# alvinwan/neural-backed-decision-trees

Measured on AMD Instinct MI355X. Metric: images/sec training SoftNBDT WRN28x10 CIFAR10, higher is better.
Workload: dtype bf16; 1 GPU; WideResNet-28-10 + SoftTreeSupLoss (induced-wrn28_10_cifar10, 10 leaves), CIFAR10-shaped 3x32x32, SGD m=0.9 wd=5e-4; batch_per_gpu=512, global_batch=512, parallelism=dp1

## Files before the change

### include/nbdt_hip.h

```cpp
#ifndef NBDT_HIP_H
#define NBDT_HIP_H

#include <stdint.h>

#ifdef __cplusplus
extern "C" {
#endif

#define NBDT_OK 0
#define NBDT_EINVAL (-1)
#define NBDT_EHIP (-2)
#define NBDT_ENOMEM (-3)

#define NBDT_F32 0
#define NBDT_BF16 1
#define NBDT_F16 2

const char* nbdt_last_error(void);
const char* nbdt_debug_last_igemm(void);
const char* nbdt_debug_last_igemm_full(void);
const char* nbdt_debug_last_wgrad(void);
int nbdt_version(void);
int nbdt_set_deterministic(int32_t on);
int nbdt_get_deterministic(void);
int nbdt_set_wgrad_store_epilogue(int32_t on);
int nbdt_get_wgrad_store_epilogue(void);
int nbdt_set_reserved_cus(int32_t n);
int nbdt_get_reserved_cus(void);
int nbdt_set_stream_nt_min_bytes(int64_t bytes);
int64_t nbdt_get_stream_nt_min_bytes(void);
int nbdt_debug_last_stream_nt(void);
int nbdt_device_count(void);

int nbdt_weight_tile_batched(const void* src_bf16, const int64_t* table, int32_t n, int64_t total_tiles,
                             void* dst_bf16, void* stream);

typedef struct nbdt_tree nbdt_tree;
int nbdt_tree_create(int device, int num_classes, int num_inodes, int root,
                     const int32_t* node_off, const int32_t* slot_off, const int32_t* slot_cls,
                     const int32_t* cls_off, const int32_t* cls_slot, const int32_t* slot_next,
                     nbdt_tree** out);
int nbdt_tree_destroy(nbdt_tree* t);
int nbdt_tree_max_depth(const nbdt_tree* t);


int nbdt_soft_forward(const nbdt_tree* t, const void* z, int ztype, int64_t B, int64_t ldz,
                      float* P, void* stream);
int nbdt_soft_backward(const nbdt_tree* t, const void* z, int ztype, int64_t B, int64_t ldz,
                       const float* gP, float* gz, void* stream);
int nbdt_soft_tree_loss(const nbdt_tree* t, const void* z, int ztype, int64_t B, int64_t ldz,
                        const int64_t* y, float w_xent, float w_tree, float grad_scale,
                        float* row_loss, float* loss, float* gz, void* stream);
int nbdt_head_soft_tree_loss(const nbdt_tree* t, const float* pooled, const float* W, const float* bias, int64_t B,
                             int32_t K, const int64_t* y, float w_xent, float w_tree, float grad_scale,
                             float* row_loss, float* loss, float* z_out, float* gpooled, float* gW, float* gb,
                             void* stream);

int nbdt_hard_tree_loss(const nbdt_tree* t, const void* z, int ztype, int64_t B, int64_t ldz,
                        const int64_t* y, float w_xent, float w_node, float grad_scale,
                        float* row_loss, float* loss, float* gz, void* stream);
int nbdt_soft_tree_loss_ex(const nbdt_tree* t, const void* z, int ztype, int64_t B, int64_t ldz, const int64_t* y,
                           const float* tprob, int64_t ldt, float smoothing, float w_xent, float w_tree,
                           float grad_scale, float* row_loss, float* loss, float* gz, void* stream);
int nbdt_hard_tree_loss_ex(const nbdt_tree* t, const void* z, int ztype, int64_t B, int64_t ldz, const int64_t* y,
                           float smoothing, float w_xent, float w_node, float grad_scale, float* row_loss, float* loss,
                           float* gz, void* stream);
int nbdt_node_logits_backward(const nbdt_tree* t, const float* gs, int64_t B, float* gz, void* stream);
int nbdt_hard_forward(const nbdt_tree* t, const void* z, int ztype, int64_t B, int64_t ldz,
                      int64_t* pred, float* onehot, int32_t* path_node, int32_t* path_child,
                      float* path_prob, float* path_entropy, void* stream);
int nbdt_node_outputs(const nbdt_tree* t, const void* z, int ztype, int64_t B, int64_t ldz,
                      float* logits, float* probs, int64_t* preds, float* entropy, void* stream);

typedef struct nbdt_tree_stats {
  int64_t* totals;
  int64_t* confusion_net;
  int64_t* confusion_hard;
  int64_t* confusion_soft;
  int64_t* node_counts;
  int64_t* node_entropy;
  int64_t* first_error_depth;
} nbdt_tree_stats;
int nbdt_tree_stats_accumulate(const nbdt_tree* t, const void* z, int ztype, int64_t B, int64_t ldz,
                               const int64_t* y, const nbdt_tree_stats* stats, float* scores, void* stream);

typedef struct nbdt_conv_desc {
  int32_t B, gh, gw;
  int32_t cin, cout;
  int32_t ntaps;
  int32_t tap_off[9];
  int32_t w_tap[9];
  int32_t w_ntaps;
  int32_t in_bs, in_hs, in_ws, in_base;
  int32_t out_bs, out_hs, out_ws, out_base;
  int32_t accumulate;
  int32_t wide_tile;
  int32_t ksplit;
  uint64_t w_tiled;
} nbdt_conv_desc;
int nbdt_conv_plan(const nbdt_conv_desc* d, int32_t* form, int32_t* ksplit);
int nbdt_conv_igemm(const nbdt_conv_desc* d, const void* in, const void* w, void* out,
                    const void* residual, void* stream);

int nbdt_conv_igemm_multi(const nbdt_conv_desc* descs, int32_t n, const void* in, const void* w, void* out,
                          void* stream);

typedef struct nbdt_conv_seg_slice {
  int32_t tensor;
  int32_t ch0;
  int32_t ntaps;
  int32_t tap[9];
  int32_t w_matrix;
  int32_t w_off[9];
} nbdt_conv_seg_slice;
typedef struct nbdt_conv_seg_class {
  int32_t nslices;
  const nbdt_conv_seg_slice* slices;
  int32_t out_bs, out_hs, out_ws, out_base;
} nbdt_conv_seg_class;
#define NBDT_SEG_MAX_SLICES 64
typedef struct nbdt_conv_seg_desc {
  int32_t B, gh, gw;
  int32_t cout;
  int32_t ntensors;
  int32_t pix_stride[4];
  int32_t nmatrices;
  int32_t w_row_stride[4];
  int32_t nclasses;
  nbdt_conv_seg_class cls[4];
  int32_t tile;
  int32_t nbuf;
} nbdt_conv_seg_desc;
int nbdt_conv_seg_create(const nbdt_conv_seg_desc* d, void** plan);
int nbdt_conv_seg_destroy(void* plan);
int nbdt_conv_seg_info(void* plan, int32_t* tile, int32_t* nbuf, int32_t* steps, int32_t* max_rounds,
                       int64_t* w_tile_elems);
int nbdt_conv_seg_tile_weights(void* plan, const void* const* w, void* w_tiles, void* stream);
int nbdt_conv_seg(void* plan, const void* const* in, const void* w_tiles, void* out, const void* residual,
                  float* bn_partials, void* stream);
int nbdt_conv_seg_steps(void* plan, int32_t cls, int32_t* out8, int32_t max_steps, int32_t* npro);

int nbdt_conv_igemm_stats(const nbdt_conv_desc* d, const void* in, const void* w, void* out,
                          const void* residual, float* bn_partials, void* stream);

int nbdt_conv_igemm_bnbwd(const nbdt_conv_desc* d, const void* in, const void* w, void* out,
                          const void* bn_x, const float* save_mean, const float* save_rstd,
                          const float* gamma, const float* beta, float* bn_partials, void* stream);
int nbdt_conv_igemm_affine(const nbdt_conv_desc* d, const void* in, const void* w, void* out,
                           const void* residual, const float* scale, const float* shift, int32_t act,
                           void* stream);

int nbdt_conv_pw(const nbdt_conv_desc* d, const void* in, const void* w, void* out,
                 float* bn_partials , void* stream);

typedef struct nbdt_wgrad_desc {
  int32_t B, gh, gw;
  int32_t cin, cout;
  int32_t ntaps;
  int32_t tap_off[9];
  int32_t w_tap[9];
  int32_t w_ntaps;
  int32_t x_bs, x_hs, x_ws, x_base;
  int32_t g_bs, g_hs, g_ws, g_base;
  int32_t variant;
  int32_t cu_budget;
} nbdt_wgrad_desc;
int nbdt_conv_wgrad(const nbdt_wgrad_desc* d, const void* x, const void* gy, float* dw,
                    void* stream);
int nbdt_conv_wgrad_blocks(const nbdt_wgrad_desc* d);

int nbdt_weight_prep(const float* w, int32_t cout, int32_t taps, int32_t cin, void* w_bf16,
                     void* wd_bf16, void* stream);

int nbdt_weight_prep_batched(const float* flat, const int64_t* table, int32_t n_layers, int64_t total_tiles,
                             void* wd_flat, void* stream);

#define NBDT_BN_SLOTS 32
int nbdt_bn_stats(const void* x, int32_t B, int32_t H, int32_t W, int32_t C, float eps,
                  float momentum, float* running_mean, float* running_var, float* scratch,
                  float* save_mean, float* save_rstd, void* stream);
int nbdt_bn_finalize(int32_t B, int32_t H, int32_t W, int32_t C, float eps, float momentum,
                     float* running_mean, float* running_var, const float* bn_partials, float* save_mean,
                     float* save_rstd, void* stream);
int nbdt_bn_apply(const void* x, const float* save_mean, const float* save_rstd, const float* gamma,
                  const float* beta, const void* residual, int32_t relu, int32_t B, int32_t H,
                  int32_t W, int32_t C, void* y, void* stream);
int nbdt_bn_apply_s2d(const void* x, const float* save_mean, const float* save_rstd, const float* gamma,
                      const float* beta, int32_t relu, int32_t B, int32_t H, int32_t W, int32_t C, void* y,
                      void* stream);
int nbdt_bn_bwd_reduce(const void* gy, const void* y, const void* x, const float* save_mean,
                       const float* save_rstd, const float* gamma, const float* beta, int32_t relu,
                       int32_t B, int32_t H, int32_t W, int32_t C, float* scratch, float* dsum,
                       float* dgamma, float* dbeta, void* stream);
int nbdt_bn_bwd_fold(int32_t B, int32_t H, int32_t W, int32_t C, const float* bn_partials, float* dsum,
                     float* dgamma, float* dbeta, void* stream);
int nbdt_bn_bwd_apply(const void* gy, const void* y, const void* x, const float* save_mean,
                      const float* save_rstd, const float* gamma, const float* beta, const float* dsum,
                      const void* gx_add, int32_t relu, int32_t B, int32_t H, int32_t W, int32_t C,
                      void* gx, void* g_resid, void* stream);
int nbdt_bn_bwd_apply_cus(const void* gy, const void* x, const float* save_mean, const float* save_rstd,
                          const float* gamma, const float* beta, const float* dsum, const void* gx_add,
                          int32_t B, int32_t H, int32_t W, int32_t C, void* gx, int32_t cus, void* stream);
int nbdt_bn_bwd_reduce_cus(const void* gy, const void* x, const float* save_mean, const float* save_rstd,
                           const float* gamma, const float* beta, int32_t B, int32_t H, int32_t W, int32_t C,
                           float* scratch, float* dsum, float* dgamma, float* dbeta, int32_t cus, void* stream);
int nbdt_bn_bwd_cus(const void* gy, const void* x, const float* save_mean, const float* save_rstd, const float* gamma,
                    const float* beta, const void* gx_add, int32_t B, int32_t H, int32_t W, int32_t C, float* slots,
                    float* slots_other, float* dsum, float* dgamma, float* dbeta, void* gx, int32_t cus,
                    void* stream);
int nbdt_bn_relu_pool(const void* x, const float* save_mean, const float* save_rstd,
                      const float* gamma, const float* beta, int32_t B, int32_t H, int32_t W,
                      int32_t C, float* pooled, void* stream);
int nbdt_pool_bn_bwd_reduce(const float* gpooled, const void* x, const float* save_mean,
                            const float* save_rstd, const float* gamma, const float* beta,
                            int32_t B, int32_t H, int32_t W, int32_t C, float* scratch, float* dsum,
                            float* dgamma, float* dbeta, void* stream);
int nbdt_pool_bn_bwd_apply(const float* gpooled, const void* x, const float* save_mean,
                           const float* save_rstd, const float* gamma, const float* beta,
                           const float* dsum, int32_t B, int32_t H, int32_t W, int32_t C, void* gx,
                           void* stream);

#define NBDT_ACT_NONE 0
#define NBDT_ACT_RELU 1
#define NBDT_ACT_SWISH 2
int nbdt_bn_act_apply(const void* x, const float* save_mean, const float* save_rstd, const float* gamma,
                      const float* beta, int32_t act, const float* gate, const void* residual, int32_t B,
                      int32_t H, int32_t W, int32_t C, void* y, void* stream);
int nbdt_bn_act_pool(const void* x, const float* save_mean, const float* save_rstd, const float* gamma,
                     const float* beta, int32_t act, const void* mul, float scale, int32_t B, int32_t H,
                     int32_t W, int32_t C, float* out, void* stream);
int nbdt_bn_act_bwd(const void* gu, const float* gate, const float* gpool, const void* x,
                    const float* save_mean, const float* save_rstd, const float* gamma, const float* beta,
                    int32_t act, const void* gx_add, int32_t B, int32_t H, int32_t W, int32_t C,
                    float* scratch, float* dsum, float* dgamma, float* dbeta, void* gx, void* stream);
int nbdt_dwconv_fwd(const void* x, const float* w, int32_t B, int32_t H, int32_t W, int32_t C, int32_t k,
                    int32_t stride, void* y, float* bn_scratch , void* stream);
int nbdt_dwconv_bwd_data(const void* gy, const float* w, int32_t B, int32_t H, int32_t W, int32_t C,
                         int32_t k, int32_t stride, void* gx, void* stream);
int nbdt_dwconv_bwd_data_bn(const void* gy, const float* w, int32_t B, int32_t H, int32_t W, int32_t C, int32_t k,
                            void* gx, const void* bn_x, const float* save_mean, const float* save_rstd,
                            const float* gamma, const float* beta, float* scratch, void* stream);
int nbdt_bn_act_bwd_apply(const void* gu, const void* x, const float* save_mean, const float* save_rstd,
                          const float* gamma, const float* beta, int32_t act, const void* gx_add, int32_t B, int32_t H,
                          int32_t W, int32_t C, float* scratch, float* dsum, float* dgamma, float* dbeta, void* gx,
                          void* stream);
int nbdt_bn_act_se_sums(const void* gu, const void* x, const float* save_mean, const float* save_rstd,
                        const float* gamma, const float* beta, int32_t act, int32_t B, int32_t H, int32_t W, int32_t C,
                        float* sums, void* stream);
int nbdt_bn_act_se_bwd_apply(const void* gu, const float* gate, const float* gpool, float* sums, const void* x,
                             const float* save_mean, const float* save_rstd, const float* gamma, const float* beta,
                             int32_t act, int32_t B, int32_t H, int32_t W, int32_t C, float* dsum, float* dgamma,
                             float* dbeta, void* gx, void* stream);
int nbdt_dwconv_bwd_weight(const void* x, const void* gy, int32_t B, int32_t H, int32_t W, int32_t C,
                           int32_t k, int32_t stride, float* dw, void* stream);
int nbdt_se_gate_fwd(const float* pooled, const float* w1, const float* b1, const float* w2,
                     const float* b2, int32_t B, int32_t C, int32_t C_real, int32_t S, float* pre1,
                     float* gate, void* stream);
int nbdt_se_gate_bwd(const float* dgate, const float* gate, const float* pre1, const float* pooled,
                     const float* w1, const float* w2, int32_t B, int32_t C, int32_t C_real, int32_t S,
                     float* dpre2, float* dpre1, float* gpool, float* dw1, float* db1, float* dw2,
                     float* db2, void* stream);
int nbdt_se_param_grad(const float* dpre2, const float* dpre1, const float* pre1, const float* pooled,
                       int32_t B, int32_t C, int32_t C_real, int32_t S, float* dw1, float* db1, float* dw2,
                       float* db2, void* stream);
int nbdt_dropout_fwd(const float* x, int64_t n, float p, uint32_t seed, uint8_t* mask, float* y,
                     void* stream);
int nbdt_dropout_bwd(const float* gy, int64_t n, float p, const uint8_t* mask, float* gx, void* stream);

int nbdt_bn_act_apply_rows(const void* x, const float* save_mean, const float* save_rstd, const float* gamma,
                           const float* beta, int32_t act, const float* gate, const void* residual,
                           const float* row_scale, int32_t B, int32_t H, int32_t W, int32_t C, void* y, void* stream);
int nbdt_bn_act_bwd_rows(const void* gu, const float* row_scale, const float* gate, const float* gpool, const void* x,
                         const float* save_mean, const float* save_rstd, const float* gamma, const float* beta,
                         int32_t act, const void* gx_add, int32_t B, int32_t H, int32_t W, int32_t C, float* scratch,
                         float* dsum, float* dgamma, float* dbeta, void* gx, void* stream);
#define NBDT_SD_MAX_UNITS 64
int nbdt_stochastic_depth_draw(uint64_t seed, uint64_t stream_id, uint64_t counter, const float* prob,
                               const float* scale, int32_t U, int32_t B, float* table, void* stream);

int nbdt_ref_conv(const nbdt_conv_desc* d, const float* in, const float* w, float* out, const float* residual,
                  void* stream);
int nbdt_ref_wgrad(const nbdt_wgrad_desc* d, const float* x, const float* gy, float* dw, void* stream);
int nbdt_ref_conv_seg(void* plan, const float* const* in, const float* const* w, float* out, const float* residual,
                      void* stream);
int nbdt_ref_bn_stats(const float* x, int32_t B, int32_t H, int32_t W, int32_t C, float eps, float momentum,
                      float* running_mean, float* running_var, float* save_mean, float* save_rstd, float* partials,
                      void* stream);
int nbdt_ref_bn_apply(const float* x, const float* save_mean, const float* save_rstd, const float* gamma,
                      const float* beta, const float* residual, int32_t relu, int32_t B, int32_t H, int32_t W,
                      int32_t C, float* y, void* stream);
int nbdt_ref_bn_apply_s2d(const float* x, const float* save_mean, const float* save_rstd, const float* gamma,
                          const float* beta, int32_t relu, int32_t B, int32_t H, int32_t W, int32_t C, float* y,
                          void* stream);
int nbdt_ref_bn_bwd(const float* gy, const float* gpooled, const float* y, const float* x, const float* save_mean,
                    const float* save_rstd, const float* gamma, const float* beta, int32_t relu, const float* gx_add,
                    int32_t B, int32_t H, int32_t W, int32_t C, int32_t reduce, float* dsum, float* dgamma,
                    float* dbeta, float* gx, float* g_resid, void* stream);
int nbdt_ref_bn_relu_pool(const float* x, const float* save_mean, const float* save_rstd, const float* gamma,
                          const float* beta, int32_t B, int32_t H, int32_t W, int32_t C, float* pooled, void* stream);
int nbdt_ref_stem_conv(const float* img, const float* w, int32_t B, int32_t H, int32_t W, int32_t cout_real,
                       int32_t cpad, int32_t stride, float* out, void* stream);
int nbdt_ref_stem_wgrad(const float* img, const float* gy, int32_t B, int32_t H, int32_t W, int32_t cout_real,
                        int32_t cpad, int32_t stride, float* dw, void* stream);
int nbdt_ref_bn_act_apply(const float* x, const float* save_mean, const float* save_rstd, const float* gamma,
                          const float* beta, int32_t act, const float* gate, const float* residual, int32_t B, int32_t H,
                          int32_t W, int32_t C, float* y, void* stream);
int nbdt_ref_bn_act_pool(const float* x, const float* save_mean, const float* save_rstd, const float* gamma,
                         const float* beta, int32_t act, const float* mul, float scale, int32_t B, int32_t H, int32_t W,
                         int32_t C, float* out, void* stream);
int nbdt_ref_bn_act_bwd(const float* gu, const float* gate, const float* gpool, const float* x, const float* save_mean,
                        const float* save_rstd, const float* gamma, const float* beta, int32_t act, const float* gx_add,
                        int32_t B, int32_t H, int32_t W, int32_t C, float* dsum, float* dgamma, float* dbeta, float* gx,
                        void* stream);
int nbdt_ref_bn_act_apply_rows(const float* x, const float* save_mean, const float* save_rstd, const float* gamma,
                               const float* beta, int32_t act, const float* gate, const float* residual,
                               const float* row_scale, int32_t B, int32_t H, int32_t W, int32_t C, float* y,
                               void* stream);
int nbdt_ref_bn_act_bwd_rows(const float* gu, const float* row_scale, const float* gate, const float* gpool,
                             const float* x, const float* save_mean, const float* save_rstd, const float* gamma,
                             const float* beta, int32_t act, const float* gx_add, int32_t B, int32_t H, int32_t W,
                             int32_t C, float* dsum, float* dgamma, float* dbeta, float* gx, void* stream);
int nbdt_ref_dwconv_fwd(const float* x, const float* w, int32_t B, int32_t H, int32_t W, int32_t C, int32_t k,
// ... 159 lines not shown
```

### neural-backed-decision-trees_amd/csrc/bn.hip

```cpp
#include "common.h"

using namespace nbdt;

constexpr int kSlots = NBDT_BN_SLOTS;
constexpr int kMaxThreads = 256;

struct Layout {
  int c8, py, threads;
};
static Layout layout_for(int C) {
  Layout l;
  l.c8 = C / 8;
  l.py = kMaxThreads / l.c8;
  if (l.py < 1) l.py = 1;
  l.threads = l.c8 * l.py;
  return l;
}
static int grid_for(const PadGeom& g, const Layout& l, int pixels_per_thread) {
  long long want = ((long long)g.npix + (long long)l.py * pixels_per_thread - 1) / ((long long)l.py * pixels_per_thread);
  if (want < 1) want = 1;
  if (want > 2048) want = 2048;
  return (int)want;
}

template <int NQ>
__device__ __forceinline__ void block_fold_to_slots(float (&acc)[NQ][8], int cx, int py, int c8, int PY, int C,
                                                    float* scratch, float* lds, unsigned slot_mask) {
  float* mine = lds + ((size_t)py * c8 + cx) * (NQ * 8);
#pragma unroll
  for (int q = 0; q < NQ; ++q)
#pragma unroll
    for (int i = 0; i < 8; ++i) mine[q * 8 + i] = acc[q][i];
  __syncthreads();
  const int nch = c8 * 8, nthr = c8 * PY;
  for (int o = py * c8 + cx; o < NQ * nch; o += nthr) {
    const int q = o / nch, c = o - q * nch;
    const float* src = lds + (size_t)(c >> 3) * (NQ * 8) + q * 8 + (c & 7);
    float s = 0.f;
    for (int r = 0; r < PY; ++r) s += src[(size_t)r * c8 * (NQ * 8)];
    atomicAdd(scratch + ((size_t)(blockIdx.x & slot_mask) * NQ + q) * C + c, s);
  }
}

__global__ __launch_bounds__(kMaxThreads) void bn_stats_kernel(const bf16_t* __restrict__ x, PadGeom g, int c8,
                                                               int PY, float* __restrict__ scratch,
                                                               unsigned slot_mask) {
  extern __shared__ float lds[];
  const int cx = threadIdx.x % c8, py = threadIdx.x / c8;
  float acc[2][8];
#pragma unroll
  for (int i = 0; i < 8; ++i) acc[0][i] = acc[1][i] = 0.f;
  for (int p = blockIdx.x * PY + py; p < g.npix; p += gridDim.x * PY) {
    const u32x4_t v = *(const u32x4_t*)(x + pad_offset(g, p) + cx * 8);
    float f[8];
    unpack8(v, f);
#pragma unroll
    for (int i = 0; i < 8; ++i) {
      acc[0][i] += f[i];
      acc[1][i] += f[i] * f[i];
    }
  }
  block_fold_to_slots<2>(acc, cx, py, c8, PY, g.C, scratch, lds, slot_mask);
}

__global__ __launch_bounds__(256) void bn_finalize_kernel(float* __restrict__ scratch, int C, float n,
                                                          float eps, float momentum,
                                                          float* __restrict__ running_mean,
                                                          float* __restrict__ running_var,
                                                          float* __restrict__ save_mean,
                                                          float* __restrict__ save_rstd) {
  for (int c = blockIdx.x * 256 + threadIdx.x; c < C; c += gridDim.x * 256) {
    float s = 0.f, sq = 0.f;
#pragma unroll 8
    for (int k = 0; k < kSlots; ++k) {
      s += scratch[((size_t)k * 2 + 0) * C + c];
      sq += scratch[((size_t)k * 2 + 1) * C + c];
    }
#pragma unroll 8
    for (int k = 0; k < kSlots; ++k) {
      scratch[((size_t)k * 2 + 0) * C + c] = 0.f;
      scratch[((size_t)k * 2 + 1) * C + c] = 0.f;
    }
    const float mean = s / n;
    float var = sq / n - mean * mean;
    var = var > 0.f ? var : 0.f;
    save_mean[c] = mean;
    save_rstd[c] = rsqrtf(var + eps);
    if (running_mean) {
      running_mean[c] = (1.f - momentum) * running_mean[c] + momentum * mean;
      const float unbiased = n > 1.f ? var * n / (n - 1.f) : var;
      running_var[c] = (1.f - momentum) * running_var[c] + momentum * unbiased;
    }
  }
}

__global__ __launch_bounds__(256) void bn_bwd_finalize_kernel(float* __restrict__ scratch, int C,
                                                              float* __restrict__ dsum,
                                                              float* __restrict__ dgamma,
                                                              float* __restrict__ dbeta) {
  for (int c = blockIdx.x * 256 + threadIdx.x; c < C; c += gridDim.x * 256) {
    float s0 = 0.f, s1 = 0.f;
#pragma unroll 8
    for (int k = 0; k < kSlots; ++k) {
      s0 += scratch[((size_t)k * 2 + 0) * C + c];
      s1 += scratch[((size_t)k * 2 + 1) * C + c];
    }
#pragma unroll 8
    for (int k = 0; k < kSlots; ++k) {
      scratch[((size_t)k * 2 + 0) * C + c] = 0.f;
      scratch[((size_t)k * 2 + 1) * C + c] = 0.f;
    }
    dsum[c] = s0;
    dsum[C + c] = s1;
    if (dbeta) dbeta[c] += s0;
    if (dgamma) dgamma[c] += s1;
  }
}

template <bool RELU, bool HAS_RES, bool NT>
__global__ __launch_bounds__(kMaxThreads) void bn_apply_kernel(const bf16_t* __restrict__ x,
                                                               const float* __restrict__ mean,
                                                               const float* __restrict__ rstd,
                                                               const float* __restrict__ gamma,
                                                               const float* __restrict__ beta,
                                                               const bf16_t* __restrict__ res, PadGeom g, int c8,
                                                               int PY, bf16_t* __restrict__ y) {
  const int cx = threadIdx.x % c8, py = threadIdx.x / c8;
  float sc[8], sh[8];
#pragma unroll
  for (int i = 0; i < 8; ++i) {
    const int c = cx * 8 + i;
    sc[i] = gamma[c] * rstd[c];
    sh[i] = beta[c] - mean[c] * sc[i];
  }
  for (int p = blockIdx.x * PY + py; p < g.npix; p += gridDim.x * PY) {
    const int o = pad_offset(g, p) + cx * 8;
    float f[8];
    unpack8(ld16_stream<NT>(x + o), f);
    float r[8];
    if (HAS_RES) unpack8(ld16_stream<NT>(res + o), r);
#pragma unroll
    for (int i = 0; i < 8; ++i) {
      float v = f[i] * sc[i] + sh[i];
      if (HAS_RES) v += r[i];
      if (RELU) v = v > 0.f ? v : 0.f;
      f[i] = v;
    }
    *(u32x4_t*)(y + o) = pack8(f);
  }
}

template <bool RELU, bool POOL>
__global__ __launch_bounds__(kMaxThreads) void bn_bwd_reduce_kernel(const bf16_t* __restrict__ gy,
                                                                    const float* __restrict__ gpooled,
                                                                    const bf16_t* __restrict__ y,
                                                                    const bf16_t* __restrict__ x,
                                                                    const float* __restrict__ mean,
                                                                    const float* __restrict__ rstd,
                                                                    const float* __restrict__ gamma,
                                                                    const float* __restrict__ beta, PadGeom g,
                                                                    int c8, int PY, float* __restrict__ scratch,
                                                                    unsigned slot_mask) {
  extern __shared__ float lds[];
  const int cx = threadIdx.x % c8, py = threadIdx.x / c8;
  const bool maskx = POOL || (RELU && y == nullptr);
  float mu[8], rs[8], sc[8], sh[8];
#pragma unroll
  for (int i = 0; i < 8; ++i) {
    const int c = cx * 8 + i;
    mu[i] = mean[c];
    rs[i] = rstd[c];
    if (maskx) { sc[i] = gamma[c] * rs[i]; sh[i] = beta[c] - mu[i] * sc[i]; }
  }
  const float inv_hw = 1.f / (float)(g.H * g.W);
  const int hw = g.H * g.W;
  float acc[2][8];
#pragma unroll
  for (int i = 0; i < 8; ++i) acc[0][i] = acc[1][i] = 0.f;
  auto one = [&](int p, const u32x4_t vx, const u32x4_t vg, const u32x4_t vy) {
    float fx[8], fg[8], fy[8];
    unpack8(vx, fx);
    if (POOL) {
      const int b = p / hw;
#pragma unroll
      for (int i = 0; i < 8; ++i) fg[i] = gpooled[(size_t)b * g.C + cx * 8 + i] * inv_hw;
    } else {
      unpack8(vg, fg);
      if (RELU && !maskx) unpack8(vy, fy);
    }
#pragma unroll
    for (int i = 0; i < 8; ++i) {
      const float xh = (fx[i] - mu[i]) * rs[i];
      float gg = fg[i];
      if (maskx) gg = (fx[i] * sc[i] + sh[i]) > 0.f ? gg : 0.f;
      else if (RELU) gg = fy[i] > 0.f ? gg : 0.f;
      acc[0][i] += gg;
      acc[1][i] += gg * xh;
    }
  };
  const int step = gridDim.x * PY;
  int p = blockIdx.x * PY + py;
  for (; p + step < g.npix; p += 2 * step) {
    const int o0 = pad_offset(g, p) + cx * 8, o1 = pad_offset(g, p + step) + cx * 8;
    const u32x4_t x0 = *(const u32x4_t*)(x + o0), x1 = *(const u32x4_t*)(x + o1);
    u32x4_t g0 = x0, g1 = x1, y0 = x0, y1 = x1;
    if (!POOL) {
      g0 = *(const u32x4_t*)(gy + o0); g1 = *(const u32x4_t*)(gy + o1);
      if (RELU && !maskx) { y0 = *(const u32x4_t*)(y + o0); y1 = *(const u32x4_t*)(y + o1); }
    }
    one(p, x0, g0, y0);
    one(p + step, x1, g1, y1);
  }
  if (p < g.npix) {
    const int o0 = pad_offset(g, p) + cx * 8;
    const u32x4_t x0 = *(const u32x4_t*)(x + o0);
    u32x4_t g0 = x0, y0 = x0;
    if (!POOL) {
      g0 = *(const u32x4_t*)(gy + o0);
      if (RELU && !maskx) y0 = *(const u32x4_t*)(y + o0);
    }
    one(p, x0, g0, y0);
  }
  block_fold_to_slots<2>(acc, cx, py, c8, PY, g.C, scratch, lds, slot_mask);
}

template <bool RELU, bool POOL, bool HAS_ADD, bool HAS_GRES>
__global__ __launch_bounds__(kMaxThreads) void bn_bwd_apply_kernel(
    const bf16_t* __restrict__ gy, const float* __restrict__ gpooled, const bf16_t* __restrict__ y,
    const bf16_t* __restrict__ x, const float* __restrict__ mean, const float* __restrict__ rstd,
    const float* __restrict__ gamma, const float* __restrict__ beta, const float* __restrict__ dsum,
    const bf16_t* __restrict__ gx_add, PadGeom g, int c8, int PY, bf16_t* __restrict__ gx,
    bf16_t* __restrict__ g_resid) {
  const int cx = threadIdx.x % c8, py = threadIdx.x / c8;
  const float inv_n = 1.f / (float)g.npix;
  const bool maskx = POOL || (RELU && y == nullptr);
  float mu[8], rs[8], sh[8], k0[8], k1[8], sc[8];
#pragma unroll
  for (int i = 0; i < 8; ++i) {
    const int c = cx * 8 + i;
    mu[i] = mean[c];
    rs[i] = rstd[c];
    sc[i] = gamma[c] * rs[i];
    if (maskx) sh[i] = beta[c] - mu[i] * sc[i];
    k0[i] = dsum[c] * inv_n;
    k1[i] = dsum[g.C + c] * inv_n;
  }
  const float inv_hw = 1.f / (float)(g.H * g.W);
  const int hw = g.H * g.W;
  auto one = [&](int p, int o, const u32x4_t vx, const u32x4_t vg, const u32x4_t vy, const u32x4_t va) {
    float fx[8], fg[8], fy[8], fa[8];
    unpack8(vx, fx);
    if (POOL) {
      const int b = p / hw;
#pragma unroll
      for (int i = 0; i < 8; ++i) fg[i] = gpooled[(size_t)b * g.C + cx * 8 + i] * inv_hw;
    } else {
      unpack8(vg, fg);
      if (RELU && !maskx) unpack8(vy, fy);
    }
    if (HAS_ADD) unpack8(va, fa);
    float out[8];
#pragma unroll
    for (int i = 0; i < 8; ++i) {
      const float xh = (fx[i] - mu[i]) * rs[i];
      float gg = fg[i];
      if (maskx) gg = (fx[i] * sc[i] + sh[i]) > 0.f ? gg : 0.f;
      else if (RELU) gg = fy[i] > 0.f ? gg : 0.f;
      fg[i] = gg;
      float v = sc[i] * (gg - k0[i] - xh * k1[i]);
      if (HAS_ADD) v += fa[i];
      out[i] = v;
    }
    *(u32x4_t*)(gx + o) = pack8(out);
    if (HAS_GRES) *(u32x4_t*)(g_resid + o) = pack8(fg);
  };
  auto load = [&](int o, u32x4_t& vx, u32x4_t& vg, u32x4_t& vy, u32x4_t& va) {
    vx = *(const u32x4_t*)(x + o);
    vg = vx; vy = vx; va = vx;
    if (!POOL) {
      vg = *(const u32x4_t*)(gy + o);
      if (RELU && !maskx) vy = *(const u32x4_t*)(y + o);
    }
    if (HAS_ADD) va = *(const u32x4_t*)(gx_add + o);
  };
  const int step = gridDim.x * PY;
  int p = blockIdx.x * PY + py;
  for (; p + step < g.npix; p += 2 * step) {
    const int o0 = pad_offset(g, p) + cx * 8, o1 = pad_offset(g, p + step) + cx * 8;
    u32x4_t x0, g0, y0, a0, x1, g1, y1, a1;
    load(o0, x0, g0, y0, a0);
    load(o1, x1, g1, y1, a1);
    one(p, o0, x0, g0, y0, a0);
    one(p + step, o1, x1, g1, y1, a1);
  }
  if (p < g.npix) {
    const int o0 = pad_offset(g, p) + cx * 8;
    u32x4_t x0, g0, y0, a0;
    load(o0, x0, g0, y0, a0);
    one(p, o0, x0, g0, y0, a0);
  }
}
// ... 76 lines not shown
    const u32x4_t x0 = ld16_stream<NT>(x + o0), g0 = ld16_stream<NT>(gy + o0);
    u32x4_t a0 = x0;
    if (HAS_ADD) a0 = ld16_stream<NT>(gx_add + o0);
    one(x0, g0, a0, o0);
  }
}

template <bool NT>
__global__ __launch_bounds__(1024) void bn_bwd_reduce_cus_kernel(const bf16_t* __restrict__ gy,
                                                                 const bf16_t* __restrict__ x,
                                                                 const float* __restrict__ mean,
                                                                 const float* __restrict__ rstd,
                                                                 const float* __restrict__ gamma,
                                                                 const float* __restrict__ beta, PadGeom g, int c8,
                                                                 int PY, float* __restrict__ scratch,
                                                                 unsigned slot_mask) {
  extern __shared__ float lds[];
  const int cx = threadIdx.x % c8, py = threadIdx.x / c8;
  const bool live = py < PY;
  float mu[8], rs[8], sc[8], sh[8];
#pragma unroll
  for (int i = 0; i < 8; ++i) {
    const int c = (live ? cx : 0) * 8 + i;
    mu[i] = mean[c];
    rs[i] = rstd[c];
    sc[i] = gamma[c] * rs[i];
    sh[i] = beta[c] - mu[i] * sc[i];
  }
  float acc[2][8];
#pragma unroll
  for (int i = 0; i < 8; ++i) acc[0][i] = acc[1][i] = 0.f;
  auto one = [&](const u32x4_t vx, const u32x4_t vg) {
    float fx[8], fg[8];
    unpack8(vx, fx);
    unpack8(vg, fg);
#pragma unroll
    for (int i = 0; i < 8; ++i) {
      const float xh = (fx[i] - mu[i]) * rs[i];
      const float gg = (fx[i] * sc[i] + sh[i]) > 0.f ? fg[i] : 0.f;
      acc[0][i] += gg;
      acc[1][i] += gg * xh;
    }
  };
  if (live) {
    const int step = gridDim.x * PY;
    int p = blockIdx.x * PY + py;
    for (; p + (kCusInFlight - 1) * step < g.npix; p += kCusInFlight * step) {
      u32x4_t vx[kCusInFlight], vg[kCusInFlight];
#pragma unroll
      for (int u = 0; u < kCusInFlight; ++u) {
        const int o = pad_offset(g, p + u * step) + cx * 8;
        vx[u] = ld16_stream<NT>(x + o);
        vg[u] = ld16_stream<NT>(gy + o);
      }
#pragma unroll
      for (int u = 0; u < kCusInFlight; ++u) one(vx[u], vg[u]);
    }
    for (; p < g.npix; p += step) {
      const int o0 = pad_offset(g, p) + cx * 8;
      one(ld16_stream<NT>(x + o0), ld16_stream<NT>(gy + o0));
    }
  }
  if (live) {
    float* mine = lds + ((size_t)py * c8 + cx) * 16;
#pragma unroll
    for (int i = 0; i < 8; ++i) { mine[i] = acc[0][i]; mine[8 + i] = acc[1][i]; }
  }
  __syncthreads();
  for (int e = threadIdx.x; e < c8 * 16; e += 1024) {
    const int which = e / (c8 * 8), c = e - which * (c8 * 8);
    float s = 0.f;
    for (int r = 0; r < PY; ++r) s += lds[((size_t)r * c8 + (c >> 3)) * 16 + which * 8 + (c & 7)];
    atomicAdd(scratch + ((size_t)(blockIdx.x & slot_mask) * 2 + which) * g.C + c, s);
  }
}

__global__ __launch_bounds__(256) void bn_relu_pool_kernel(const bf16_t* __restrict__ x,
                                                           const float* __restrict__ mean,
                                                           const float* __restrict__ rstd,
                                                           const float* __restrict__ gamma,
                                                           const float* __restrict__ beta, PadGeom g,
                                                           float* __restrict__ pooled) {
  const int c8 = g.C / 8;
  const int idx = blockIdx.x * 256 + threadIdx.x;
  if (idx >= g.B * c8) return;
  const int b = idx / c8, cx = idx - b * c8;
  float sc[8], sh[8], acc[8];
#pragma unroll
  for (int i = 0; i < 8; ++i) {
    const int c = cx * 8 + i;
    sc[i] = gamma[c] * rstd[c];
    sh[i] = beta[c] - mean[c] * sc[i];
    acc[i] = 0.f;
  }
  for (int h = 0; h < g.H; ++h)
    for (int w = 0; w < g.W; ++w) {
      float f[8];
      unpack8(*(const u32x4_t*)(x + (size_t)b * g.img + (h + 1) * g.row + (w + 1) * g.C + cx * 8), f);
#pragma unroll
      for (int i = 0; i < 8; ++i) {
        const float v = f[i] * sc[i] + sh[i];
        acc[i] += v > 0.f ? v : 0.f;
      }
    }
  const float inv = 1.f / (float)(g.H * g.W);
#pragma unroll
  for (int i = 0; i < 8; ++i) pooled[(size_t)b * g.C + cx * 8 + i] = acc[i] * inv;
}


static int check_shape(int B, int H, int W, int C) {
  NBDT_REQUIRE(B > 0 && H > 0 && W > 0 && C > 0, "empty tensor");
  NBDT_REQUIRE(C % 8 == 0 && C / 8 <= kMaxThreads, "C must be a multiple of 8 and <= 2048");
  NBDT_REQUIRE((long long)B * (H + 2) * (W + 2) * C < (1ll << 31), "tensor too large for 32-bit offsets");
  return NBDT_OK;
}


struct SlotTarget {
  float* ptr;
  unsigned mask;
  bool det;
};
static int slot_target(hipStream_t st, float* scratch, int grid, size_t n, SlotTarget* t) {
  t->ptr = scratch; t->mask = kSlots - 1; t->det = false;
  if (!deterministic()) return NBDT_OK;
  float* rows = det_rows(st, (size_t)grid * n);
  if (!rows) return nbdt::fail(NBDT_ENOMEM, "deterministic mode: %s (%s)", "no workspace for the per-block rows", nbdt::det_rows_why());
  NBDT_HIP_CHECK(hipMemsetAsync(rows, 0, (size_t)grid * n * sizeof(float), st));
  t->ptr = rows; t->mask = ~0u; t->det = true;
  return NBDT_OK;
}
static int slot_finish(hipStream_t st, const SlotTarget& t, int grid, size_t n, float* scratch) {
  return t.det ? det_fold(st, t.ptr, grid, n, scratch) : NBDT_OK;
}

extern "C" int nbdt_bn_stats(const void* x, int32_t B, int32_t H, int32_t W, int32_t C, float eps, float momentum,
                             float* running_mean, float* running_var, float* scratch, float* save_mean,
                             float* save_rstd, void* stream) {
  NBDT_REQUIRE(scratch && save_mean && save_rstd, "null argument");
  NBDT_REQUIRE((running_mean == nullptr) == (running_var == nullptr), "running stats must be both set or both NULL");
  int rc = check_shape(B, H, W, C);
  if (rc) return rc;
  hipStream_t st = (hipStream_t)stream;
  const PadGeom g = make_geom(B, H, W, C);
  if (x != nullptr) {
    const Layout l = layout_for(C);
    const size_t shmem = (size_t)l.threads * 16 * sizeof(float);
    const int grid = grid_for(g, l, 16);
    SlotTarget t;
    rc = slot_target(st, scratch, grid, 2 * (size_t)C, &t);
    if (rc) return rc;
    hipLaunchKernelGGL(bn_stats_kernel, dim3(grid), dim3(l.threads), shmem, st, (const bf16_t*)x, g,
                       l.c8, l.py, t.ptr, t.mask);
    NBDT_LAUNCH_CHECK();
    rc = slot_finish(st, t, grid, 2 * (size_t)C, scratch);
    if (rc) return rc;
  }
  hipLaunchKernelGGL(bn_finalize_kernel, dim3((C + 255) / 256), dim3(256), 0, st, scratch, C, (float)g.npix, eps, momentum,
                     running_mean, running_var, save_mean, save_rstd);
  NBDT_LAUNCH_CHECK();
  return NBDT_OK;
}

template <int CL>
__global__ __launch_bounds__(1024) void bn_fold_partials_kernel(const float* __restrict__ part, int rows, int C,
                                                                float n, float eps, float momentum,
                                                                float* __restrict__ running_mean,
                                                                float* __restrict__ running_var,
                                                                float* __restrict__ save_mean,
                                                                float* __restrict__ save_rstd) {
  constexpr int RL = 1024 / CL;
  static_assert(CL <= 32 && 64 % CL == 0, "a wave holds whole groups of CL channels");
  __shared__ float red[2][16][CL + 1];
  const int cl = threadIdx.x % CL, rs = threadIdx.x / CL;
  const int c = blockIdx.x * CL + cl;
  float s0 = 0.f, s1 = 0.f, s2 = 0.f, s3 = 0.f, q0 = 0.f, q1 = 0.f, q2 = 0.f, q3 = 0.f;
  if (c < C) {
    int r = rs;
    for (; r + 3 * RL < rows; r += 4 * RL) {
      s0 += part[((size_t)r * 2 + 0) * C + c];             q0 += part[((size_t)r * 2 + 1) * C + c];
      s1 += part[((size_t)(r + RL) * 2 + 0) * C + c];      q1 += part[((size_t)(r + RL) * 2 + 1) * C + c];
      s2 += part[((size_t)(r + 2 * RL) * 2 + 0) * C + c];  q2 += part[((size_t)(r + 2 * RL) * 2 + 1) * C + c];
      s3 += part[((size_t)(r + 3 * RL) * 2 + 0) * C + c];  q3 += part[((size_t)(r + 3 * RL) * 2 + 1) * C + c];
    }
    for (; r < rows; r += RL) {
      s0 += part[((size_t)r * 2 + 0) * C + c];
      q0 += part[((size_t)r * 2 + 1) * C + c];
    }
  }
  float ws = (s0 + s1) + (s2 + s3), wq = (q0 + q1) + (q2 + q3);
#pragma unroll
  for (int off = CL; off < 64; off <<= 1) {
    ws += __shfl_xor(ws, off, 64);
    wq += __shfl_xor(wq, off, 64);
  }
  const int lane = threadIdx.x & 63, wave = threadIdx.x >> 6;
  if (lane < CL) { red[0][wave][lane] = ws; red[1][wave][lane] = wq; }
  __syncthreads();
  if (rs == 0 && c < C) {
    float s = 0.f, sq = 0.f;
#pragma unroll
    for (int k = 0; k < 16; ++k) { s += red[0][k][cl]; sq += red[1][k][cl]; }
    const float mean = s / n;
    float var = sq / n - mean * mean;
    var = var > 0.f ? var : 0.f;
    save_mean[c] = mean;
    save_rstd[c] = rsqrtf(var + eps);
    if (running_mean) {
      running_mean[c] = (1.f - momentum) * running_mean[c] + momentum * mean;
      const float unbiased = n > 1.f ? var * n / (n - 1.f) : var;
      running_var[c] = (1.f - momentum) * running_var[c] + momentum * unbiased;
    }
  }
}

__global__ __launch_bounds__(1024) void bn_bwd_fold_partials_kernel(const float* __restrict__ part, int rows, int C,
                                                                    float* __restrict__ dsum,
                                                                    float* __restrict__ dgamma,
                                                                    float* __restrict__ dbeta) {
  __shared__ float red[2][32][33];
  const int cl = threadIdx.x & 31, rs = threadIdx.x >> 5;
  const int c = blockIdx.x * 32 + cl;
  float s0 = 0.f, s1 = 0.f, q0 = 0.f, q1 = 0.f;
  if (c < C) {
    int r = rs;
    for (; r + 32 < rows; r += 64) {
      s0 += part[((size_t)r * 2 + 0) * C + c];         q0 += part[((size_t)r * 2 + 1) * C + c];
      s1 += part[((size_t)(r + 32) * 2 + 0) * C + c];  q1 += part[((size_t)(r + 32) * 2 + 1) * C + c];
    }
    for (; r < rows; r += 32) {
      s0 += part[((size_t)r * 2 + 0) * C + c];
      q0 += part[((size_t)r * 2 + 1) * C + c];
    }
  }
  red[0][rs][cl] = s0 + s1;
  red[1][rs][cl] = q0 + q1;
  __syncthreads();
  if (rs == 0 && c < C) {
    float a = 0.f, b = 0.f;
    for (int k = 0; k < 32; ++k) { a += red[0][k][cl]; b += red[1][k][cl]; }
    dsum[c] = a;
    dsum[C + c] = b;
    if (dbeta) dbeta[c] += a;
    if (dgamma) dgamma[c] += b;
  }
}

extern "C" int nbdt_bn_bwd_fold(int32_t B, int32_t H, int32_t W, int32_t C, const float* bn_partials, float* dsum,
                                float* dgamma, float* dbeta, void* stream) {
  NBDT_REQUIRE(bn_partials && dsum, "null argument");
  int rc = check_shape(B, H, W, C);
  if (rc) return rc;
  const int rows = (int)(((long long)B * H * W + 255) / 256);
  hipLaunchKernelGGL(bn_bwd_fold_partials_kernel, dim3((C + 31) / 32), dim3(1024), 0, (hipStream_t)stream, bn_partials,
                     rows, C, dsum, dgamma, dbeta);
  NBDT_LAUNCH_CHECK();
  return NBDT_OK;
}

extern "C" int nbdt_bn_finalize(int32_t B, int32_t H, int32_t W, int32_t C, float eps, float momentum,
                                float* running_mean, float* running_var, const float* partials, float* save_mean,
                                float* save_rstd, void* stream) {
  NBDT_REQUIRE(partials && save_mean && save_rstd, "null argument");
  NBDT_REQUIRE((running_mean == nullptr) == (running_var == nullptr), "running stats must be both set or both NULL");
  int rc = check_shape(B, H, W, C);
  if (rc) return rc;
  const long long npix = (long long)B * H * W;
  const int rows = (int)((npix + 255) / 256);
  if (rows >= 1024)
    hipLaunchKernelGGL(bn_fold_partials_kernel<8>, dim3((C + 7) / 8), dim3(1024), 0, (hipStream_t)stream, partials, rows,
                       C, (float)npix, eps, momentum, running_mean, running_var, save_mean, save_rstd);
  else
    hipLaunchKernelGGL(bn_fold_partials_kernel<32>, dim3((C + 31) / 32), dim3(1024), 0, (hipStream_t)stream, partials,
                       rows, C, (float)npix, eps, momentum, running_mean, running_var, save_mean, save_rstd);
  NBDT_LAUNCH_CHECK();
  return NBDT_OK;
}

extern "C" int nbdt_bn_apply(const void* x, const float* save_mean, const float* save_rstd, const float* gamma,
                             const float* beta, const void* residual, int32_t relu, int32_t B, int32_t H, int32_t W,
                             int32_t C, void* y, void* stream) {
  NBDT_REQUIRE(x && save_mean && save_rstd && gamma && beta && y, "null argument");
  int rc = check_shape(B, H, W, C);
  if (rc) return rc;
  hipStream_t st = (hipStream_t)stream;
  const PadGeom g = make_geom(B, H, W, C);
  const Layout l = layout_for(C);
  const dim3 grid(grid_for(g, l, 8)), blk(l.threads);
  const bool nt = stream_nt((long long)B * g.img * 2);
#define NBDT_APPLY(R, S)                                                                                         \
  do {                                                                                                           \
    if (nt) hipLaunchKernelGGL((bn_apply_kernel<R, S, true>), grid, blk, 0, st, (const bf16_t*)x, save_mean, save_rstd, gamma, \
                               beta, (const bf16_t*)residual, g, l.c8, l.py, (bf16_t*)y);                          \
    else hipLaunchKernelGGL((bn_apply_kernel<R, S, false>), grid, blk, 0, st, (const bf16_t*)x, save_mean, save_rstd, gamma, \
                            beta, (const bf16_t*)residual, g, l.c8, l.py, (bf16_t*)y);                             \
  } while (0)
  if (relu) { if (residual) NBDT_APPLY(true, true); else NBDT_APPLY(true, false); }
  else { if (residual) NBDT_APPLY(false, true); else NBDT_APPLY(false, false); }
#undef NBDT_APPLY
  NBDT_LAUNCH_CHECK();
  return NBDT_OK;
}

template <bool RELU>
__global__ __launch_bounds__(kMaxThreads) void bn_apply_s2d_kernel(const bf16_t* __restrict__ x,
                                                                   const float* __restrict__ mean,
                                                                   const float* __restrict__ rstd,
                                                                   const float* __restrict__ gamma,
                                                                   const float* __restrict__ beta, PadGeom g, int c8,
                                                                   int PY, bf16_t* __restrict__ y) {
  const int cx = threadIdx.x % c8, py = threadIdx.x / c8;
  float sc[8], sh[8];
#pragma unroll
  for (int i = 0; i < 8; ++i) {
    const int c = cx * 8 + i;
    sc[i] = gamma[c] * rstd[c];
    sh[i] = beta[c] - mean[c] * sc[i];
  }
  const int row2 = (g.W / 2 + 2) * 4 * g.C, img2 = (g.H / 2 + 2) * row2;
  for (int p = blockIdx.x * PY + py; p < g.npix; p += gridDim.x * PY) {
    const unsigned t = fdiv((unsigned)p, g.div_w);
    const int w = p - (int)t * g.W;
    const unsigned b = fdiv(t, g.div_h);
    const int h = (int)t - (int)b * g.H;
    const int o = (int)b * g.img + (h + 1) * g.row + (w + 1) * g.C + cx * 8;
    const int o2 = (int)b * img2 + ((h >> 1) + 1) * row2 + ((w >> 1) + 1) * 4 * g.C + ((h & 1) * 2 + (w & 1)) * g.C + cx * 8;
    float f[8];
    unpack8(*(const u32x4_t*)(x + o), f);
#pragma unroll
    for (int i = 0; i < 8; ++i) {
      float v = f[i] * sc[i] + sh[i];
      if (RELU) v = v > 0.f ? v : 0.f;
      f[i] = v;
    }
    *(u32x4_t*)(y + o2) = pack8(f);
  }
}

extern "C" int nbdt_bn_apply_s2d(const void* x, const float* save_mean, const float* save_rstd, const float* gamma,
                                 const float* beta, int32_t relu, int32_t B, int32_t H, int32_t W, int32_t C, void* y,
                                 void* stream) {
  NBDT_REQUIRE(x && save_mean && save_rstd && gamma && beta && y, "null argument");
  NBDT_REQUIRE(H % 2 == 0 && W % 2 == 0, "space-to-depth needs even H and W");
  int rc = check_shape(B, H, W, C);
  if (rc) return rc;
  hipStream_t st = (hipStream_t)stream;
  const PadGeom g = make_geom(B, H, W, C);
  const Layout l = layout_for(C);
  const dim3 grid(grid_for(g, l, 8)), blk(l.threads);
  if (relu)
    hipLaunchKernelGGL((bn_apply_s2d_kernel<true>), grid, blk, 0, st, (const bf16_t*)x, save_mean, save_rstd, gamma,
                       beta, g, l.c8, l.py, (bf16_t*)y);
  else
    hipLaunchKernelGGL((bn_apply_s2d_kernel<false>), grid, blk, 0, st, (const bf16_t*)x, save_mean, save_rstd, gamma,
                       beta, g, l.c8, l.py, (bf16_t*)y);
  NBDT_LAUNCH_CHECK();
  return NBDT_OK;
}

extern "C" int nbdt_bn_bwd_reduce(const void* gy, const void* y, const void* x, const float* save_mean,
                                  const float* save_rstd, const float* gamma, const float* beta, int32_t relu,
                                  int32_t B, int32_t H, int32_t W, int32_t C, float* scratch, float* dsum,
                                  float* dgamma, float* dbeta, void* stream) {
  NBDT_REQUIRE(gy && x && save_mean && save_rstd && scratch && dsum, "null argument");
  NBDT_REQUIRE(!relu || y || (gamma && beta), "relu backward needs y, or gamma+beta to recompute the mask");
  int rc = check_shape(B, H, W, C);
  if (rc) return rc;
  hipStream_t st = (hipStream_t)stream;
  const PadGeom g = make_geom(B, H, W, C);
  const Layout l = layout_for(C);
  const size_t shmem = (size_t)l.threads * 16 * sizeof(float);
  const int nblk = grid_for(g, l, 16);
  const dim3 grid(nblk), blk(l.threads);
  SlotTarget t;
  rc = slot_target(st, scratch, nblk, 2 * (size_t)C, &t);
  if (rc) return rc;
  if (relu)
    hipLaunchKernelGGL((bn_bwd_reduce_kernel<true, false>), grid, blk, shmem, st, (const bf16_t*)gy, nullptr,
                       (const bf16_t*)y, (const bf16_t*)x, save_mean, save_rstd, gamma, beta, g, l.c8, l.py,
                       t.ptr, t.mask);
  else
    hipLaunchKernelGGL((bn_bwd_reduce_kernel<false, false>), grid, blk, shmem, st, (const bf16_t*)gy, nullptr,
                       (const bf16_t*)y, (const bf16_t*)x, save_mean, save_rstd, gamma, beta, g, l.c8, l.py,
                       t.ptr, t.mask);
  NBDT_LAUNCH_CHECK();
  rc = slot_finish(st, t, nblk, 2 * (size_t)C, scratch);
  if (rc) return rc;
  hipLaunchKernelGGL(bn_bwd_finalize_kernel, dim3((C + 255) / 256), dim3(256), 0, st, scratch, C, dsum, dgamma, dbeta);
  NBDT_LAUNCH_CHECK();
  return NBDT_OK;
}

extern "C" int nbdt_bn_bwd_apply(const void* gy, const void* y, const void* x, const float* save_mean,
                                 const float* save_rstd, const float* gamma, const float* beta, const float* dsum,
                                 const void* gx_add, int32_t relu, int32_t B, int32_t H, int32_t W, int32_t C,
                                 void* gx, void* g_resid, void* stream) {
  NBDT_REQUIRE(gy && x && save_mean && save_rstd && gamma && dsum && gx, "null argument");
  NBDT_REQUIRE(!relu || y || beta, "relu backward needs y, or beta to recompute the mask");
  int rc = check_shape(B, H, W, C);
  if (rc) return rc;
  hipStream_t st = (hipStream_t)stream;
  const PadGeom g = make_geom(B, H, W, C);
  const Layout l = layout_for(C);
  const dim3 grid(grid_for(g, l, 8)), blk(l.threads);
#define NBDT_BA(R, A, G)                                                                                          \
  hipLaunchKernelGGL((bn_bwd_apply_kernel<R, false, A, G>), grid, blk, 0, st, (const bf16_t*)gy, nullptr,          \
                     (const bf16_t*)y, (const bf16_t*)x, save_mean, save_rstd, gamma, beta, dsum,                  \
                     (const bf16_t*)gx_add, g, l.c8, l.py, (bf16_t*)gx, (bf16_t*)g_resid)
  const bool a = gx_add != nullptr, r = g_resid != nullptr;
  if (relu) {
    if (a) { if (r) NBDT_BA(true, true, true); else NBDT_BA(true, true, false); }
    else { if (r) NBDT_BA(true, false, true); else NBDT_BA(true, false, false); }
  } else {
    if (a) { if (r) NBDT_BA(false, true, true); else NBDT_BA(false, true, false); }
    else { if (r) NBDT_BA(false, false, true); else NBDT_BA(false, false, false); }
  }
#undef NBDT_BA
  NBDT_LAUNCH_CHECK();
  return NBDT_OK;
}

extern "C" int nbdt_bn_bwd_apply_cus(const void* gy, const void* x, const float* save_mean, const float* save_rstd,
                                    const float* gamma, const float* beta, const float* dsum, const void* gx_add,
                                    int32_t B, int32_t H, int32_t W, int32_t C, void* gx, int32_t cus,
                                    void* stream) {
  NBDT_REQUIRE(gy && x && save_mean && save_rstd && gamma && beta && dsum && gx, "null argument");
  NBDT_REQUIRE(cus >= 1 && cus <= 256, "cus must be 1..256");
  int rc = check_shape(B, H, W, C);
  if (rc) return rc;
  const PadGeom g = make_geom(B, H, W, C);
  const int c8 = C / 8;
  const int py = 1024 / c8;
  const bool nt = stream_nt((long long)B * g.img * 2);
  constexpr int kForceLds = 96 * 1024;
  static DeviceAttr site;
  if (site.need(kForceLds)) {
    NBDT_ATTR_CHECK(site, hipFuncSetAttribute(reinterpret_cast<const void*>(&bn_bwd_apply_cus_kernel<true, false, false>),
                                              hipFuncAttributeMaxDynamicSharedMemorySize, kForceLds));
    NBDT_ATTR_CHECK(site, hipFuncSetAttribute(reinterpret_cast<const void*>(&bn_bwd_apply_cus_kernel<true, false, true>),
                                              hipFuncAttributeMaxDynamicSharedMemorySize, kForceLds));
    NBDT_ATTR_CHECK(site, hipFuncSetAttribute(reinterpret_cast<const void*>(&bn_bwd_apply_cus_kernel<false, false, false>),
                                              hipFuncAttributeMaxDynamicSharedMemorySize, kForceLds));
    NBDT_ATTR_CHECK(site, hipFuncSetAttribute(reinterpret_cast<const void*>(&bn_bwd_apply_cus_kernel<false, false, true>),
                                              hipFuncAttributeMaxDynamicSharedMemorySize, kForceLds));
    site.done(kForceLds);
  }
  int blocks = cus;
  const int max_blocks = (g.npix + py - 1) / py;
// ... 178 lines not shown
```

### neural-backed-decision-trees_amd/csrc/common.h

```cpp
#pragma once
#include <hip/hip_runtime.h>
#include <hip/hip_bf16.h>
#include <hip/hip_fp16.h>
#include <stdint.h>
#include <stdio.h>
#include <string.h>

#include <mutex>

#include "../../include/nbdt_hip.h"

#if !defined(NBDT_TIMING_BUILD) &&                                                                                    \
    (defined(NBDT_EPI_TIMING) || (defined(NBDT_PP_TIMING) && (NBDT_PP_TIMING + 0) != 0) ||                            \
     (defined(NBDT_WPP_TIMING) && (NBDT_WPP_TIMING + 0) != 0) || (defined(NBDT_SEG_TIMING) && (NBDT_SEG_TIMING + 0) != 0) || \
     (defined(NBDT_RULES_TIMING) && (NBDT_RULES_TIMING + 0) != 0))
#error "timing switch without -DNBDT_TIMING_BUILD: a stamped build is not a product library (csrc/common.h)"
#endif
#ifdef NBDT_TIMING_BUILD
extern "C" __attribute__((weak, used, visibility("default"))) int nbdt_timing_build() { return 1; }
#endif

namespace nbdt {

extern thread_local char g_err[512];

inline int fail(int code, const char* fmt, const char* a = "", const char* b = "") {
  snprintf(g_err, sizeof(g_err), fmt, a, b);
  return code;
}

#define NBDT_HIP_CHECK(expr)                                                              \
  do {                                                                                    \
    hipError_t _e = (expr);                                                               \
    if (_e != hipSuccess) return nbdt::fail(NBDT_EHIP, "%s: %s", #expr, hipGetErrorString(_e)); \
  } while (0)

#define NBDT_REQUIRE(cond, msg)                                       \
  do {                                                                \
    if (!(cond)) return nbdt::fail(NBDT_EINVAL, "%s (%s)", msg, #cond); \
  } while (0)

#define NBDT_LAUNCH_CHECK() NBDT_HIP_CHECK(hipGetLastError())

struct DeviceAttr {
  static constexpr int kMaxDevices = 64;
  std::mutex m;
  size_t bytes[kMaxDevices] = {};
  int dev = 0;
  bool need(size_t want) {
    int d = 0;
    (void)hipGetDevice(&d);
    if (d < 0 || d >= kMaxDevices) d = kMaxDevices - 1;
    m.lock();
    dev = d;
    if (bytes[d] >= want && want > 0) { m.unlock(); return false; }
    return true;
  }
  void done(size_t want) { bytes[dev] = want ? want : 1; m.unlock(); }
  void abort() { m.unlock(); }
};
#define NBDT_ATTR_CHECK(site, expr)                                                       \
  do {                                                                                    \
    hipError_t _e = (expr);                                                               \
    if (_e != hipSuccess) { (site).abort(); return nbdt::fail(NBDT_EHIP, "%s: %s", #expr, hipGetErrorString(_e)); } \
  } while (0)

bool deterministic();
bool wgrad_store_epilogue();
int reserved_cus();
float* det_rows(hipStream_t st, size_t floats);
const char* det_rows_why();
int det_fold(hipStream_t st, const float* rows, int nrows, size_t n, float* dst);

typedef unsigned short bf16_t;

__device__ __forceinline__ float bf16_to_f32(bf16_t v) {
  return __uint_as_float(((unsigned)v) << 16);
}
__device__ __forceinline__ bf16_t f32_to_bf16(float f) {
  unsigned u = __float_as_uint(f);
  if ((u & 0x7fffffffu) > 0x7f800000u) return (bf16_t)((u >> 16) | 0x40);
  u += 0x7fffu + ((u >> 16) & 1u);
  return (bf16_t)(u >> 16);
}
__device__ __forceinline__ unsigned pack_bf16x2(float lo, float hi) {
  unsigned r;
  asm("v_cvt_pk_bf16_f32 %0, %1, %2" : "=v"(r) : "v"(lo), "v"(hi));
  return r;
}
__device__ __forceinline__ uint2 bf16x4_of(const float4 v) {
  uint2 o;
  o.x = pack_bf16x2(v.x, v.y);
  o.y = pack_bf16x2(v.z, v.w);
  return o;
}

template <class T>
__device__ __forceinline__ T wave_sum(T v) {
#pragma unroll
  for (int o = 32; o > 0; o >>= 1) v += __shfl_xor(v, o, 64);
  return v;
}

struct FastDiv {
  unsigned mul, sh, d;
};
inline FastDiv make_fastdiv(unsigned d) {
  FastDiv f;
  f.d = d;
  if (d == 1) { f.mul = 0; f.sh = 0; return f; }
  unsigned s = 0;
  while ((1ull << s) < d) ++s;
  const unsigned long long num = 1ull << (31 + s);
  f.mul = (unsigned)((num + d - 1) / d);
  f.sh = s - 1;
  return f;
}
__device__ __forceinline__ unsigned fdiv(unsigned n, const FastDiv& f) {
  return f.d == 1 ? n : (__umulhi(n, f.mul) >> f.sh);
}

struct PadGeom {
  int B, H, W, C;
  int npix;
  int row;
  int img;
  FastDiv div_w, div_h;
};
inline PadGeom make_geom(int B, int H, int W, int C) {
  PadGeom g;
  g.B = B; g.H = H; g.W = W; g.C = C;
  g.npix = B * H * W;
  g.row = (W + 2) * C;
  g.img = (H + 2) * g.row;
  g.div_w = make_fastdiv((unsigned)W);
  g.div_h = make_fastdiv((unsigned)H);
  return g;
}
__device__ __forceinline__ int pad_offset(const PadGeom& g, int p) {
  const unsigned t = fdiv((unsigned)p, g.div_w);
  const int w = p - (int)t * g.W;
  const unsigned b = fdiv(t, g.div_h);
  const int h = (int)t - (int)b * g.H;
  return (int)b * g.img + (h + 1) * g.row + (w + 1) * g.C;
}

int wgrad_dma(const nbdt_wgrad_desc* d, const void* x, const void* gy, float* dw, hipStream_t st);

bool wgrad_taps_applicable(const nbdt_wgrad_desc* d);
int wgrad_taps(const nbdt_wgrad_desc* d, const void* x, const void* gy, float* dw, hipStream_t st);
int wgrad_taps_blocks(const nbdt_wgrad_desc* d);

bool wgrad_s2d_applicable(const nbdt_wgrad_desc* d);
int wgrad_s2d(const nbdt_wgrad_desc* d, const void* x, const void* gy, float* dw, hipStream_t st);
int wgrad_s2d_blocks(const nbdt_wgrad_desc* d);

struct BnBwdArgs {
  const void* x;
  const float *mean, *rstd, *gamma, *beta;
  const float *aff_scale = nullptr, *aff_shift = nullptr;
  int aff_act = 0;
};
int conv_igemm_dma(const nbdt_conv_desc* d, const void* in, const void* w, void* out, const void* res,
                   float* stats, const BnBwdArgs* bn, int M, hipStream_t st);
int conv_igemm_dma_multi(const nbdt_conv_desc* descs, int n, const void* in, const void* w, void* out, hipStream_t st);

struct HaloGeom {
  int ib, rb;
  int hw2;
  int himg;
  int hp;
  int a_instr;
  int a_bytes;
  int blocks_per_img;
  int nwv;
  int mw;
  int lpitch, limg;
  int pad, dv;
  int row_magic;
};
bool conv_halo_applicable(const nbdt_conv_desc* d, int M, HaloGeom* hg);
int conv_ksplit_rule(const nbdt_conv_desc& d, int nt, int items);
int conv_halo_items(const nbdt_conv_desc& d, const HaloGeom& hg, int M, int* nt_out);
extern thread_local const char* g_last_wgrad;
extern thread_local const char* g_last_igemm;
extern thread_local char g_last_igemm_full[128];
struct BnBwdArgs;
int conv3x3_halo(const nbdt_conv_desc* d, const HaloGeom& hg, const void* in, const void* w, void* out,
                 const void* res, float* stats, const BnBwdArgs* bn, int M, hipStream_t st);

}

__device__ __forceinline__ void glds16_s(const void* sbase, unsigned voff, unsigned lds_dst) {
  unsigned keep;
  asm volatile(
      "s_mov_b32 %0, m0\n\t"
      "s_mov_b32 m0, %3\n\t"
      "s_nop 2\n\t"
      "global_load_lds_dwordx4 %1, %2\n\t"
      "s_mov_b32 m0, %0"
      : "=&s"(keep)
      : "v"(voff), "s"(sbase), "s"(lds_dst)
      : "memory");
}

__device__ __forceinline__ void glds16_sf(const void* sbase, unsigned voff, unsigned lds_dst) {
  const unsigned long long b = (unsigned long long)sbase;
  const unsigned lo = __builtin_amdgcn_readfirstlane((unsigned)b), hi = __builtin_amdgcn_readfirstlane((unsigned)(b >> 32));
  glds16_s((const void*)(((unsigned long long)hi << 32) | lo), voff, __builtin_amdgcn_readfirstlane(lds_dst));
}

namespace nbdt {

typedef __attribute__((ext_vector_type(4))) unsigned u32x4_t;

template <bool NT>
__device__ __forceinline__ u32x4_t ld16_stream(const void* p) {
  if (NT) return __builtin_nontemporal_load((const u32x4_t*)p);
  return *(const u32x4_t*)p;
}
constexpr int kStreamNtMinMiB = 96;
bool stream_nt(long long tensor_bytes);

template <bool WT = true>
__device__ __forceinline__ void st16(void* p, const u32x4_t v) {
  if (WT) asm volatile("global_store_dwordx4 %0, %1, off sc1\n\ts_nop 2" ::"v"(p), "v"(v) : "memory");
  else *(u32x4_t*)p = v;
}

__device__ __forceinline__ void unpack8(const u32x4_t v, float* f) {
#pragma unroll
  for (int i = 0; i < 4; ++i) {
    f[2 * i] = __uint_as_float(v[i] << 16);
    f[2 * i + 1] = __uint_as_float(v[i] & 0xffff0000u);
  }
}
__device__ __forceinline__ u32x4_t pack8(const float* f) {
  u32x4_t v;
#pragma unroll
  for (int i = 0; i < 4; ++i) v[i] = pack_bf16x2(f[2 * i], f[2 * i + 1]);
  return v;
}

}
```

### neural-backed-decision-trees_amd/csrc/rules.hip

```cpp
#include "common.h"

#include <algorithm>
#include <vector>

namespace nbdt {
thread_local char g_err[512] = "";
}

using namespace nbdt;

struct nbdt_tree {
  int device;
  int cus;
  int C, N, R, L, root, max_depth;
  int sched_len;
  int32_t* d_all;
  const int32_t *node_off, *slot_off, *slot_cls, *cls_off, *cls_slot, *slot_next;
  const int32_t* sched;
};

struct TreeView {
  int C, N, R, L, root, max_depth, sched_len;
  int tl_ints;
  int staged;
// ... 1124 lines not shown
    if (t.staged) ga.issue(t.slot_cls, t.L, active, g_tid);
    load_and_node_logits<TPS, LD>(t, o, z, sample * ldz, active, g_tid, zs, ss, stage, ga, gb,
                                  want_soft ? t.cls_slot : nullptr);
    node_softmax<TPS>(t, o, active, g_tid, ss, ps);
    int64_t yy = -1;
    if (active && a.y != nullptr) yy = a.y[sample];
    const bool valid = yy >= 0 && yy < t.C;

    if (active)
      for (int n = g_tid; n < t.N; n += TPS) {
        const int b = o.node_off[n], e = o.node_off[n + 1];
        int best = b;
        for (int s = b + 1; s < e; ++s)
          if (ss[s] > ss[best]) best = s;
        info[n] = best;
        next_of[n] = t.slot_next[best];
        if (valid && a.node_entropy != nullptr) {
          const float h = node_entropy(ps, b, e);
          atomicAdd(ent + 2 * n, entropy_fixed(h));
          atomicAdd(ent + 2 * n + 1, entropy_fixed(h * h));
        }
      }

    float vz = -INFINITY;
    int iz = 0x7fffffff;
    if (active)
      for (int c = g_tid; c < t.C; c += TPS)
        if (zs[c] > vz) { vz = zs[c]; iz = c; }
    group_argmax<TPS>(vz, iz, red, g_tid);
    float h_net = 0.f, top_diff = 0.f;
    if (want_scores) {
      float sum = 0.f, v2 = -INFINITY;
      if (active)
        for (int c = g_tid; c < t.C; c += TPS) {
          sum += expf(zs[c] - vz);
          if (c != iz) v2 = fmaxf(v2, zs[c]);
        }
      sum = group_sum<TPS>(sum, red, g_tid);
      v2 = group_max<TPS>(v2, red, g_tid);
      const float eps = 1.1920928955078125e-07f;
      float h = 0.f;
      if (active)
        for (int c = g_tid; c < t.C; c += TPS) {
          const float p = expf(zs[c] - vz) / sum;
          h += p * logf(fminf(fmaxf(p, eps), 1.0f - eps));
        }
      h_net = -group_sum<TPS>(h, red, g_tid);
      top_diff = 1.0f / sum - expf(v2 - vz) / sum;
    }
    __syncthreads();

    if (valid) {
      const int pb = o.cls_off[yy], pe = o.cls_off[yy + 1];
      for (int j = pb + g_tid; j < pe; j += TPS) {
        const int s = t.cls_slot[j];
        int lo = 0, hi = t.N - 1;
        while (lo < hi) {
          const int mid = (lo + hi + 1) >> 1;
          if (o.node_off[mid] <= s) lo = mid; else hi = mid - 1;
        }
        const int b = o.node_off[lo], e = o.node_off[lo + 1];
        if (j > pb && t.cls_slot[j - 1] >= b) continue;
        const int best = info[lo];
        bool right = s == best;
        for (int jj = j + 1; jj < pe && !right; ++jj) {
          const int s2 = t.cls_slot[jj];
          if (s2 >= e) break;
          right = s2 == best;
        }
        info[lo] = best | kOnPath | (right ? kRight : 0);
        if (a.node_counts != nullptr) {
          lds_count(cnt + 5 * lo);
          if (right) lds_count(cnt + 5 * lo + 1);
        }
      }
    }
    __syncthreads();
    if (want_soft) stage_paths<TPS>(t, ps, stage, g_tid, gb);

    int hard_cls = -1, first_err = t.max_depth;
    float spread = 0.f;
    if (active && g_tid == TPS - 1) {
      int n = t.root;
      float emax = 0.f, emin = 0.f;
      for (int d = 0; d < t.max_depth; ++d) {
        const int inf = info[n];
        if (valid && a.node_counts != nullptr) {
          lds_count(cnt + 5 * n + 2);
          if (inf & kOnPath) lds_count(cnt + 5 * n + 3);
          if (inf & kRight) lds_count(cnt + 5 * n + 4);
        }
        if (first_err == t.max_depth && !(inf & kRight)) first_err = d;
        if (want_scores) {
          const float h = node_entropy(ps, o.node_off[n], o.node_off[n + 1]);
          emax = fmaxf(emax, h);
          emin = fminf(emin, h);
        }
        const int nx = next_of[n];
        if (nx < 0) { hard_cls = -nx - 1; break; }
        n = nx;
      }
      spread = emax - emin;
    }

    float vp = -INFINITY;
    int ip = 0x7fffffff;
    if (want_soft) {
      if (active)
        for (int c0 = g_tid; c0 < t.C; c0 += joint_of<TPS>() * TPS) {
          float p[joint_of<TPS>()];
          class_chains<TPS, ChainMul>(t, o, c0, ps, stage, 1.0f, p);
#pragma unroll
          for (int m = 0; m < joint_of<TPS>(); ++m)
            if (c0 + m * TPS < t.C && p[m] > vp) { vp = p[m]; ip = c0 + m * TPS; }
        }
      group_argmax<TPS>(vp, ip, red, g_tid);
    }

    if (active && g_tid == TPS - 1) {
      if (valid) {
        lds_count(tot);
        if (iz == yy) lds_count(tot + 1);
        if (hard_cls == yy) lds_count(tot + 2);
        if (want_soft && ip == yy) lds_count(tot + 3);
        lds_count(fed + first_err);
        const int64_t row = yy * t.C;
        if (a.conf_net != nullptr && iz >= 0 && iz < t.C) add_i64(a.conf_net + row + iz, 1);
        if (a.conf_hard != nullptr && hard_cls >= 0 && hard_cls < t.C) add_i64(a.conf_hard + row + hard_cls, 1);
        if (a.conf_soft != nullptr && ip >= 0 && ip < t.C) add_i64(a.conf_soft + row + ip, 1);
      }
      if (want_scores) {
        a.scores[sample * 3] = h_net;
        a.scores[sample * 3 + 1] = top_diff;
        a.scores[sample * 3 + 2] = spread;
      }
    }
    __syncthreads();
  }

  if (a.node_counts != nullptr)
    for (int i = threadIdx.x; i < 5 * t.N; i += (int)blockDim.x)
      if (cnt[i] != 0) add_i64(a.node_counts + i, cnt[i]);
  if (a.totals != nullptr && threadIdx.x < 4 && tot[threadIdx.x] != 0) add_i64(a.totals + threadIdx.x, tot[threadIdx.x]);
  if (a.first_error != nullptr)
    for (int i = threadIdx.x; i <= t.max_depth; i += (int)blockDim.x)
      if (fed[i] != 0) add_i64(a.first_error + i, fed[i]);
  if (a.node_entropy != nullptr)
    for (int i = threadIdx.x; i < 2 * t.N; i += (int)blockDim.x)
      if (ent[i] != 0ull) add_i64(a.node_entropy + i, (long long)ent[i]);
}


extern "C" const char* nbdt_last_error(void) { return nbdt::g_err; }
extern "C" int nbdt_version(void) { return 124; }
extern "C" int nbdt_device_count(void) {
  int n = 0;
  if (hipGetDeviceCount(&n) != hipSuccess) return 0;
  return n;
}

static int pick_tps(int C, int R) { return (C <= 64 && R <= 64) ? 64 : (C <= 512 && R <= 512) ? 256 : 1024; }

static void build_slot_schedule(int R, const int32_t* slot_off, int lanes, std::vector<int32_t>* out, int* len) {
  std::vector<int> order(R);
  for (int s = 0; s < R; ++s) order[s] = s;
  auto length = [&](int s) { return slot_off[s + 1] - slot_off[s]; };
  std::stable_sort(order.begin(), order.end(), [&](int a, int b) { return length(a) > length(b); });
  const int waves = lanes / 64, chunks = (R + 63) / 64;
  std::vector<std::vector<int>> mine(waves);
  std::vector<long> load(waves, 0);
  for (int c = 0; c < chunks; ++c) {
    const int longest = length(order[c * 64]);
    int w = 0;
    for (int i = 1; i < waves; ++i)
      if (load[i] < load[w]) w = i;
    mine[w].push_back(c);
    load[w] += 64 + 8L * longest;
  }
  size_t rows = 0;
  for (auto& m : mine) rows = std::max(rows, m.size());
  const int n = (int)rows * lanes;
  out->assign((size_t)3 * n, -1);
  for (int w = 0; w < waves; ++w)
    for (size_t k = 0; k < mine[w].size(); ++k)
      for (int l = 0; l < 64; ++l) {
        const int i = mine[w][k] * 64 + l;
        if (i >= R) break;
        const int at = (int)k * lanes + w * 64 + l, s = order[i];
        (*out)[at] = s;
        (*out)[n + at] = slot_off[s];
        (*out)[2 * n + at] = slot_off[s + 1];
      }
  *len = n;
}

extern "C" int nbdt_tree_create(int device, int C, int N, int root, const int32_t* node_off,
                                const int32_t* slot_off, const int32_t* slot_cls, const int32_t* cls_off,
                                const int32_t* cls_slot, const int32_t* slot_next, nbdt_tree** out) {
  NBDT_REQUIRE(out && node_off && slot_off && slot_cls && cls_off && cls_slot && slot_next, "null argument");
  NBDT_REQUIRE(C > 0 && N > 0 && root >= 0 && root < N, "bad tree sizes");
  const int R = node_off[N];
  const int L = slot_off[R];
  NBDT_REQUIRE(R > 0 && L > 0 && cls_off[C] == L, "inconsistent CSR maps");
  for (int n = 0; n < N; ++n) NBDT_REQUIRE(node_off[n + 1] > node_off[n], "inner node without children");
  for (int s = 0; s < R; ++s) {
    NBDT_REQUIRE(slot_off[s + 1] > slot_off[s], "child without leaves");
    NBDT_REQUIRE(slot_next[s] < N && slot_next[s] >= -C, "bad slot_next");
  }
  for (int j = 0; j < L; ++j) {
    NBDT_REQUIRE(slot_cls[j] >= 0 && slot_cls[j] < C, "class index out of range");
    NBDT_REQUIRE(cls_slot[j] >= 0 && cls_slot[j] < R, "slot index out of range");
  }
  for (int c = 0; c < C; ++c)
    for (int j = cls_off[c] + 1; j < cls_off[c + 1]; ++j)
      NBDT_REQUIRE(cls_slot[j] > cls_slot[j - 1], "cls_slot must list a class's slots in ascending order");
  int max_depth = 0;
  {
    int* depth = new int[N];
    for (int n = 0; n < N; ++n) depth[n] = 1;
    bool changed = true;
    int iters = 0;
    while (changed && iters <= N + 1) {
      changed = false;
      ++iters;
      for (int n = 0; n < N; ++n)
        for (int s = node_off[n]; s < node_off[n + 1]; ++s)
          if (slot_next[s] >= 0 && depth[n] < depth[slot_next[s]] + 1) {
            depth[n] = depth[slot_next[s]] + 1;
            changed = true;
          }
    }
    max_depth = depth[root];
    delete[] depth;
    NBDT_REQUIRE(iters <= N + 1, "hierarchy has a cycle");
  }

  int prev = 0;
  NBDT_HIP_CHECK(hipGetDevice(&prev));
  NBDT_HIP_CHECK(hipSetDevice(device));
  int cus = 0;
  if (hipDeviceGetAttribute(&cus, hipDeviceAttributeMultiprocessorCount, device) != hipSuccess || cus <= 0) cus = 1;
  std::vector<int32_t> sched;
  int sched_len = 0;
  build_slot_schedule(R, slot_off, pick_tps(C, R), &sched, &sched_len);
  nbdt_tree* t = new nbdt_tree();
  t->device = device; t->cus = cus; t->C = C; t->N = N; t->R = R; t->L = L; t->root = root; t->max_depth = max_depth;
  t->sched_len = sched_len;
  const size_t n_ints = (size_t)(N + 1) + (R + 1) + L + (C + 1) + L + R + sched.size();
  hipError_t e = hipMalloc((void**)&t->d_all, n_ints * sizeof(int32_t));
  if (e != hipSuccess) {
    delete t;
    (void)hipSetDevice(prev);
    return nbdt::fail(NBDT_ENOMEM, "hipMalloc(tree): %s", hipGetErrorString(e));
  }
  int32_t* host = new int32_t[n_ints];
  size_t o = 0;
  auto put = [&](const int32_t* src, size_t n, const int32_t** dst) {
    memcpy(host + o, src, n * sizeof(int32_t));
    *dst = t->d_all + o;
    o += n;
  };
  put(node_off, N + 1, &t->node_off);
  put(slot_off, R + 1, &t->slot_off);
  put(slot_cls, L, &t->slot_cls);
  put(cls_off, C + 1, &t->cls_off);
  put(cls_slot, L, &t->cls_slot);
  put(slot_next, R, &t->slot_next);
  put(sched.data(), sched.size(), &t->sched);
  e = hipMemcpy(t->d_all, host, n_ints * sizeof(int32_t), hipMemcpyHostToDevice);
  delete[] host;
  (void)hipSetDevice(prev);
  if (e != hipSuccess) {
    (void)hipFree(t->d_all);
    delete t;
    return nbdt::fail(NBDT_EHIP, "hipMemcpy(tree): %s", hipGetErrorString(e));
  }
  *out = t;
  return NBDT_OK;
}

extern "C" int nbdt_tree_destroy(nbdt_tree* t) {
  if (!t) return NBDT_OK;
  (void)hipFree(t->d_all);
  delete t;
  return NBDT_OK;
}

extern "C" int nbdt_tree_max_depth(const nbdt_tree* t) { return t ? t->max_depth : 0; }

static int pick_tps(const nbdt_tree* t) { return pick_tps(t->C, t->R); }

constexpr size_t kLdsBytes = 160 * 1024;
constexpr size_t kStagePad = 4;

template <typename... KA, typename... A>
static int launch_rules(void (*kernel)(KA...), unsigned grid, int block, size_t shmem, hipStream_t st,
                        A... args) {
  if (shmem > 64 * 1024)
    NBDT_HIP_CHECK(hipFuncSetAttribute(reinterpret_cast<const void*>(kernel),
                                       hipFuncAttributeMaxDynamicSharedMemorySize, (int)shmem));
  hipLaunchKernelGGL(kernel, dim3(grid), dim3(block), shmem, st, args...);
  NBDT_LAUNCH_CHECK();
  return NBDT_OK;
}

#define NBDT_DISPATCH_RULES_EX(KERNEL, NEXT, BASE_FLOATS, BLOCK_INTS, BLOCKS_PER_CU, ...)                  \
  do {                                                                                               \
// ... 245 lines not shown
```

### neural-backed-decision-trees_amd/csrc/wgrad.hip

```cpp
#include "common.h"

using namespace nbdt;

extern "C" int nbdt_conv_wgrad(const nbdt_wgrad_desc* d, const void* x, const void* gy, float* dw,
                               void* stream) {
  NBDT_REQUIRE(d && x && gy && dw, "null argument");
  NBDT_REQUIRE(d->cin > 0 && d->cin % 32 == 0 && d->cout > 0 && d->cout % 32 == 0, "channels must be multiples of 32");
  NBDT_REQUIRE(d->ntaps >= 1 && d->ntaps <= 9 && d->w_ntaps >= 1, "bad tap table");
  NBDT_REQUIRE(d->B > 0 && d->gh > 0 && d->gw > 0, "empty pixel grid");
  for (int t = 0; t < d->ntaps; ++t) {
    NBDT_REQUIRE(d->w_tap[t] >= 0 && d->w_tap[t] < d->w_ntaps, "bad w_tap");
    NBDT_REQUIRE(d->tap_off[t] % 8 == 0, "tap offsets must be 16-byte aligned");
  }
  NBDT_REQUIRE(d->x_bs % 8 == 0 && d->x_hs % 8 == 0 && d->x_ws % 8 == 0 && d->x_base % 8 == 0 &&
               d->g_bs % 8 == 0 && d->g_hs % 8 == 0 && d->g_ws % 8 == 0 && d->g_base % 8 == 0,
               "pixel offsets must be 16-byte aligned");
  NBDT_REQUIRE(d->cu_budget == 0 || (d->cu_budget >= 32 && d->cu_budget <= 256), "cu_budget must be 0 or 32..256");
  const int64_t M_all = (int64_t)d->B * d->gh * d->gw;
  NBDT_REQUIRE(M_all < (1ll << 31), "pixel grid too large");
  if (nbdt::wgrad_taps_applicable(d)) return nbdt::wgrad_taps(d, x, gy, dw, (hipStream_t)stream);
  if (d->variant != 3 && nbdt::wgrad_s2d_applicable(d)) return nbdt::wgrad_s2d(d, x, gy, dw, (hipStream_t)stream);
  NBDT_REQUIRE(d->variant == 0 || d->variant == 3, "variant 2 / 4 / 5 select between the dense 3x3 stride-1 kernels only");
  nbdt::g_last_wgrad = "conv_wgrad_dma_kernel";
  return nbdt::wgrad_dma(d, x, gy, dw, (hipStream_t)stream);
}

extern "C" int nbdt_conv_wgrad_blocks(const nbdt_wgrad_desc* d) {
  if (!d || d->cin <= 0 || d->cin % 32 != 0 || d->cout <= 0 || d->cout % 32 != 0 || d->ntaps != 9) return 0;
  if (d->B <= 0 || d->gh <= 0 || d->gw <= 0) return 0;
  if (d->cu_budget != 0 && (d->cu_budget < 32 || d->cu_budget > 256)) return 0;
  if (d->variant != 3 && nbdt::wgrad_s2d_applicable(d)) return nbdt::wgrad_s2d_blocks(d);
  return nbdt::wgrad_taps_blocks(d);
}

namespace nbdt { thread_local const char* g_last_wgrad = ""; }
extern "C" const char* nbdt_debug_last_wgrad(void) { return nbdt::g_last_wgrad; }
```

### neural-backed-decision-trees_amd/csrc/wgrad_dma.hip

```cpp
#include "common.h"
#include <stdlib.h>

using namespace nbdt;

typedef __attribute__((ext_vector_type(8))) short bf16x8;
typedef __attribute__((ext_vector_type(4))) short s16x4;
typedef __attribute__((ext_vector_type(4))) float f32x4;

namespace nbdt {

struct WgradDmaParams {
  nbdt_wgrad_desc d;
  const bf16_t* x;
  const bf16_t* gy;
  float* dw;
  long long dw_split_stride;
  int M;
  int chunks;
  int chunks_per_split;
  int n_ci_blocks;
  int splits, items, per_xcd;
  FastDiv div_gw, div_gh;
};

}

constexpr int KS = 32;
constexpr int NSTAGE = 3;

__device__ __forceinline__ void glds16(const void* gsrc, unsigned lds_dst) {
  unsigned keep;
  asm volatile(
      "s_mov_b32 %0, m0\n\t"
      "s_mov_b32 m0, %2\n\t"
      "s_nop 0\n\t"
      "global_load_lds_dwordx4 %1, off\n\t"
      "s_mov_b32 m0, %0"
      : "=&s"(keep)
      : "v"(gsrc), "s"(lds_dst)
      : "memory");
}

constexpr int min_dma_per_wave(int g_instr, int x_instr) {
  int best = 1 << 30;
  for (int w = 0; w < 4; ++w) {
    int n = 0;
    for (int id = w; id < g_instr; id += 4) ++n;
    for (int id = (w + 2) & 3; id < x_instr; id += 4) ++n;
    best = n < best ? n : best;
  }
  return best;
}

template <int WM, int WN>
__global__ __launch_bounds__(256, 2) void conv_wgrad_dma_kernel(nbdt::WgradDmaParams p) {
  constexpr int CG = 32 * WM, CX = 32 * WN;
  constexpr int G_BYTES = (CG / 8) * 512, X_BYTES = (CX / 8) * 512;
  constexpr int STAGE = G_BYTES + X_BYTES;
  constexpr int G_INSTR = CG / 16, X_INSTR = CX / 16;
  constexpr int IPG = (G_INSTR + 3) / 4, IPX = (X_INSTR + 3) / 4;
  constexpr int MINPW = min_dma_per_wave(G_INSTR, X_INSTR);
  extern __shared__ __attribute__((aligned(16))) unsigned char smem[];

  const nbdt_wgrad_desc& d = p.d;
  const int tid = threadIdx.x;
  const int lane = tid & 63;
  const int wave = __builtin_amdgcn_readfirstlane(tid >> 6);
  const int wm = wave >> 1, wn = wave & 1;

  const int item = (blockIdx.x & 7) * p.per_xcd + (blockIdx.x >> 3);
  if (item >= p.items) return;
  const int tap = item % d.ntaps;
  const int rest = item / d.ntaps;
  const int split = rest % p.splits;
  const int tile = rest / p.splits;
  const int co_blk = tile / p.n_ci_blocks;
  const int ci_blk = tile - co_blk * p.n_ci_blocks;
  const int co0 = co_blk * CG;
  const int ci0 = ci_blk * CX;
  const int c_begin = split * p.chunks_per_split;
  int c_end = c_begin + p.chunks_per_split;
  c_end = c_end < p.chunks ? c_end : p.chunks;
  if (c_begin >= c_end) return;
  const int n_chunks = c_end - c_begin;

#define NBDT_PIN(x) __builtin_amdgcn_readfirstlane(x)
  const int M = NBDT_PIN(p.M);
  const int g_bs = NBDT_PIN(d.g_bs), g_hs = NBDT_PIN(d.g_hs), g_ws = NBDT_PIN(d.g_ws);
  const int x_bs = NBDT_PIN(d.x_bs), x_hs = NBDT_PIN(d.x_hs), x_ws = NBDT_PIN(d.x_ws);
  FastDiv dgw, dgh;
  dgw.mul = NBDT_PIN(p.div_gw.mul); dgw.sh = NBDT_PIN(p.div_gw.sh); dgw.d = NBDT_PIN(p.div_gw.d);
  dgh.mul = NBDT_PIN(p.div_gh.mul); dgh.sh = NBDT_PIN(p.div_gh.sh); dgh.d = NBDT_PIN(p.div_gh.d);
  const unsigned long long gy_u = (unsigned long long)p.gy, x_u = (unsigned long long)p.x;
  const bf16_t* gy_base = (const bf16_t*)(((unsigned long long)NBDT_PIN((unsigned)(gy_u >> 32)) << 32) |
                                          (unsigned)NBDT_PIN((unsigned)gy_u));
  const bf16_t* x_base = (const bf16_t*)(((unsigned long long)NBDT_PIN((unsigned)(x_u >> 32)) << 32) |
                                         (unsigned)NBDT_PIN((unsigned)x_u));
#undef NBDT_PIN

  const int hi_half = lane >> 5;
  const int my_px = (lane & 31) ^ (hi_half << 3);
  const int g_base_off = d.g_base + co0 + hi_half * 8;
  const int x_base_off = d.x_base + d.tap_off[tap] + ci0 + hi_half * 8;
  const int g_zero = co0 + hi_half * 8;
  const int x_zero = ci0 + hi_half * 8;
  const unsigned lds_base = (unsigned)(size_t)(__attribute__((address_space(3))) unsigned char*)smem;

  auto issue = [&](int slot, int chunk) {
    const int m = chunk * KS + my_px;
    const bool valid = m < M;
    const unsigned mm = valid ? (unsigned)m : 0u;
    const unsigned t1 = fdiv(mm, dgw);
    const int j = (int)(mm - t1 * dgw.d);
    const unsigned b = fdiv(t1, dgh);
    const int i = (int)(t1 - b * dgh.d);
    const int og = valid ? ((int)b * g_bs + i * g_hs + j * g_ws + g_base_off) : g_zero;
    const int ox = valid ? ((int)b * x_bs + i * x_hs + j * x_ws + x_base_off) : x_zero;
    const bf16_t* gsrc = gy_base + og;
    const bf16_t* xsrc = x_base + ox;
    const unsigned dst0 = lds_base + slot * STAGE;
#pragma unroll
    for (int k = 0; k < IPG; ++k) {
      const int id = wave + 4 * k;
      if (id < G_INSTR)
        glds16(gsrc + id * 16, __builtin_amdgcn_readfirstlane(dst0 + id * 1024));
    }
#pragma unroll
    for (int k = 0; k < IPX; ++k) {
      const int id = ((wave + 2) & 3) + 4 * k;
      if (id < X_INSTR)
        glds16(xsrc + id * 16, __builtin_amdgcn_readfirstlane(dst0 + G_BYTES + id * 1024));
    }
  };

  f32x4 acc[WM][WN];
#pragma unroll
  for (int a = 0; a < WM; ++a)
#pragma unroll
    for (int b = 0; b < WN; ++b) acc[a][b] = f32x4{0.f, 0.f, 0.f, 0.f};

  const int g4 = lane >> 4, t16 = lane & 15;
  const int rr = 4 * g4 + (t16 >> 2);
  const int q = (t16 & 3) >> 1;
  const int lane_off = q * 512 + ((rr ^ (q << 3)) << 4) + (t16 & 1) * 8;
  const int g_lane_off = lane_off + wm * WM * 1024;
  const int x_lane_off = lane_off + wn * WN * 1024;

  auto frag = [&](const unsigned char* tile_lane, int ch_tile) -> bf16x8 {
    const unsigned char* a0 = tile_lane + ch_tile * 1024;
    const s16x4 lo = __builtin_amdgcn_ds_read_tr16_b64_v4i16((__attribute__((address_space(3))) s16x4*)(a0));
    const s16x4 hi = __builtin_amdgcn_ds_read_tr16_b64_v4i16((__attribute__((address_space(3))) s16x4*)(a0 + 256));
    return bf16x8{lo[0], lo[1], lo[2], lo[3], hi[0], hi[1], hi[2], hi[3]};
  };

  auto compute = [&](int slot) {
    const unsigned char* Gs = smem + slot * STAGE + g_lane_off;
    const unsigned char* Xs = smem + slot * STAGE + G_BYTES + x_lane_off;
    bf16x8 gf[WM];
#pragma unroll
    for (int a = 0; a < WM; ++a) gf[a] = frag(Gs, a);
#pragma unroll
    for (int b = 0; b < WN; ++b) {
      const bf16x8 xf = frag(Xs, b);
#pragma unroll
      for (int a = 0; a < WM; ++a)
        acc[a][b] = __builtin_amdgcn_mfma_f32_16x16x32_bf16(gf[a], xf, acc[a][b], 0, 0, 0);
    }
  };

  issue(0, c_begin);
  if (n_chunks > 1) issue(1, c_begin + 1);
  int slot = 0;
  for (int t = 0; t < n_chunks; ++t) {
    if (t + 1 < n_chunks) {
      asm volatile("s_waitcnt vmcnt(%0) lgkmcnt(0)" ::"n"(MINPW) : "memory");
    } else {
      asm volatile("s_waitcnt vmcnt(0) lgkmcnt(0)" ::: "memory");
    }
    __builtin_amdgcn_s_barrier();
    asm volatile("" ::: "memory");
    if (t + 2 < n_chunks) {
      int s2 = slot + 2;
      s2 = s2 >= NSTAGE ? s2 - NSTAGE : s2;
      issue(s2, c_begin + t + 2);
    }
    compute(slot);
    slot = slot + 1 == NSTAGE ? 0 : slot + 1;
  }

  const int w_tap = d.w_tap[tap];
#pragma unroll
  for (int a = 0; a < WM; ++a)
#pragma unroll
    for (int b = 0; b < WN; ++b) {
      const int ci = ci0 + (wn * WN + b) * 16 + t16;
#pragma unroll
      for (int r = 0; r < 4; ++r) {
        const int co = co0 + (wm * WM + a) * 16 + 4 * g4 + r;
        atomicAdd(p.dw + (int64_t)split * p.dw_split_stride + ((int64_t)co * d.w_ntaps + w_tap) * d.cin + ci, acc[a][b][r]);
      }
    }
}

namespace nbdt {

template <int WM, int WN>
static int launch_dma(WgradDmaParams& p, hipStream_t st) {
  const nbdt_wgrad_desc& d = p.d;
  p.n_ci_blocks = d.cin / (32 * WN);
  const int tiles = d.ntaps * (d.cout / (32 * WM)) * p.n_ci_blocks;
  int splits = 512 / tiles;
  const int max_splits = p.chunks / 16 > 0 ? p.chunks / 16 : 1;
  if (splits > max_splits) splits = max_splits;
  if (splits < 1) splits = 1;
  p.chunks_per_split = (p.chunks + splits - 1) / splits;
  splits = (p.chunks + p.chunks_per_split - 1) / p.chunks_per_split;
  p.splits = splits;
  p.items = tiles * splits;
  p.per_xcd = (p.items + 7) / 8;
  const size_t shmem = (size_t)NSTAGE * (32 * WM / 8 + 32 * WN / 8) * 512;
  static DeviceAttr site;
  if (site.need(shmem)) {
    NBDT_ATTR_CHECK(site, hipFuncSetAttribute(reinterpret_cast<const void*>(&conv_wgrad_dma_kernel<WM, WN>),
                                              hipFuncAttributeMaxDynamicSharedMemorySize, (int)shmem));
    site.done(shmem);
  }
  float* const dw = p.dw;
  const size_t dw_elems = (size_t)p.d.cout * p.d.w_ntaps * p.d.cin;
  p.dw_split_stride = 0;
  if (deterministic()) {
    float* rows = det_rows(st, (size_t)p.splits * dw_elems);
    if (!rows) return nbdt::fail(NBDT_ENOMEM, "deterministic mode: %s (%s)", "no workspace for the per-split gradients", nbdt::det_rows_why());
    NBDT_HIP_CHECK(hipMemsetAsync(rows, 0, (size_t)p.splits * dw_elems * sizeof(float), st));
    p.dw = rows;
    p.dw_split_stride = (long long)dw_elems;
  }
  hipLaunchKernelGGL((conv_wgrad_dma_kernel<WM, WN>), dim3(p.per_xcd * 8), dim3(256), shmem, st, p);
  NBDT_LAUNCH_CHECK();
  if (p.dw != dw) return det_fold(st, p.dw, p.splits, dw_elems, dw);
  return NBDT_OK;
}

int wgrad_dma(const nbdt_wgrad_desc* d, const void* x, const void* gy, float* dw, hipStream_t st) {
  WgradDmaParams p;
  p.d = *d;
  p.x = (const bf16_t*)x;
  p.gy = (const bf16_t*)gy;
  p.dw = dw;
  p.M = d->B * d->gh * d->gw;
  p.chunks = (p.M + KS - 1) / KS;
  p.div_gw = make_fastdiv((unsigned)d->gw);
  p.div_gh = make_fastdiv((unsigned)d->gh);
  const int mt = d->cout / 32, nt = d->cin / 32;
#define NBDT_WG(WM_, WN_) return launch_dma<WM_, WN_>(p, st)
#define NBDT_WG_ROW(WM_)                 \
  do {                                   \
    if (nt % 5 == 0) NBDT_WG(WM_, 5);    \
    if (nt % 4 == 0) NBDT_WG(WM_, 4);    \
    if (nt % 3 == 0) NBDT_WG(WM_, 3);    \
    if (nt % 2 == 0) NBDT_WG(WM_, 2);    \
    NBDT_WG(WM_, 1);                     \
  } while (0)
  if (mt % 5 == 0) NBDT_WG_ROW(5);
  if (mt % 4 == 0) NBDT_WG_ROW(4);
  if (mt % 3 == 0) NBDT_WG_ROW(3);
  if (mt % 2 == 0) NBDT_WG_ROW(2);
  NBDT_WG_ROW(1);
#undef NBDT_WG_ROW
#undef NBDT_WG
}

}
```

### neural-backed-decision-trees_amd/csrc/wgrad_taps.hip

```cpp
#include "common.h"
#include <stdlib.h>
#include <algorithm>
#include <type_traits>

using namespace nbdt;

typedef __attribute__((ext_vector_type(8))) short bf16x8;
typedef __attribute__((ext_vector_type(4))) short s16x4;
typedef __attribute__((ext_vector_type(4))) float f32x4;
typedef __attribute__((ext_vector_type(2))) unsigned u32x2;

namespace nbdt {
struct WgradTapsParams {
  nbdt_wgrad_desc d;
  const bf16_t* x;
  const bf16_t* gy;
  float* dw;
  long long dw_split_stride;
  int stages;
  int stages_per_split;
  int n_ci_blocks;
  int splits, items, per_xcd;
  int store;
  int rs, cs;
// ... 909 lines not shown
#pragma unroll
  for (int u = 0; u < PD; ++u)
    if (u < n_st) {
      int gs, xs;
      stage_off(s_begin + u, gs, xs);
      issue(u, gs, xs);
    }
  asm volatile("s_waitcnt vmcnt(0)" ::: "memory");
  __builtin_amdgcn_s_barrier();
  for (int i = 0; i < grp; ++i) __builtin_amdgcn_s_barrier();
  __builtin_amdgcn_sched_barrier(0);

  lds_cptr xa[KK][3];
  lds_cptr ga[2];
  auto prepare = [&](int slot_i) {
    int off = slot_i * STAGE;
    asm volatile("" : "+s"(off));
    const lds_cptr base = smem3 + off;
    ga[0] = base + g_lane_off[0];
    ga[1] = base + g_lane_off[1];
#pragma unroll
    for (int kk = 0; kk < KK; ++kk)
#pragma unroll
      for (int q = 0; q < 3; ++q) xa[kk][q] = base + xrel[kk][q];
  };
  prepare(0);
  int slot_n = 1 % NSLOT, slot_d = PD % NSLOT;
  int g_next = 0, x_next = 0;
  if (PD < n_st) stage_off(s_begin + PD, g_next, x_next);

  for (int u = 0; u < n_st; ++u) {
    bf16x8 gf[KK][WM];
    u32x2 xw[KK][3];
    auto read_chunk = [&](auto kk_c) {
      constexpr int kk = decltype(kk_c)::value;
#pragma unroll
      for (int a = 0; a < WM; ++a) {
        const lds_cptr a0 = ga[a & 1] + ((a >> 1) * 64 + kk * 32 * PG);
        const s16x4 lo = __builtin_amdgcn_ds_read_tr16_b64_v4i16((lds_tr)(a0));
        const s16x4 hi = __builtin_amdgcn_ds_read_tr16_b64_v4i16((lds_tr)(a0 + 4 * PG));
        gf[kk][a] = bf16x8{lo[0], lo[1], lo[2], lo[3], hi[0], hi[1], hi[2], hi[3]};
      }
#pragma unroll
      for (int q = 0; q < 3; ++q)
        xw[kk][q] = __builtin_bit_cast(u32x2, __builtin_amdgcn_ds_read_tr16_b64_v4i16((lds_tr)xa[kk][q]));
    };
    auto x_frag = [&](int kk, int sft) {
      const u32x2 A = xw[kk][0], B = xw[kk][1], C = xw[kk][2];
      u32x4_t v;
      if (sft == 0) v = u32x4_t{A[0], A[1], B[0], B[1]};
      else if (sft == 2) v = u32x4_t{A[1], B[0], B[1], C[0]};
      else v = u32x4_t{__builtin_amdgcn_alignbit(A[1], A[0], 16), __builtin_amdgcn_alignbit(B[0], A[1], 16),
                       __builtin_amdgcn_alignbit(B[1], B[0], 16), __builtin_amdgcn_alignbit(C[0], B[1], 16)};
      return __builtin_bit_cast(bf16x8, v);
    };
    const bool dma_now = u + PD < n_st;
    read_chunk(std::integral_constant<int, 0>{});
    if (dma_now) issue(slot_d, g_next, x_next);
    {
      const int fly = (dma_now ? n_mine : 0) + (u + PD - 1 < n_st ? n_mine : 0);
      switch (fly) {
#define NBDT_CASE(K) case K: asm volatile("s_waitcnt vmcnt(%0)" ::"n"(K) : "memory"); break;
        NBDT_CASE(1) NBDT_CASE(2) NBDT_CASE(3) NBDT_CASE(4) NBDT_CASE(5) NBDT_CASE(6)
#undef NBDT_CASE
        default: asm volatile("s_waitcnt vmcnt(0)" ::: "memory"); break;
      }
    }
    asm volatile("s_waitcnt lgkmcnt(0)" ::: "memory");
    __builtin_amdgcn_sched_barrier(0);
    __builtin_amdgcn_s_barrier();
    __builtin_amdgcn_sched_barrier(0);
    read_chunk(std::integral_constant<int, 1>{});
    asm volatile("s_waitcnt lgkmcnt(0)" ::: "memory");
    __builtin_amdgcn_sched_barrier(0);
    __builtin_amdgcn_s_barrier();
    __builtin_amdgcn_sched_barrier(0);
    __builtin_amdgcn_s_setprio(1);
    prepare(slot_n);
    stage_off(s_begin + u + 1 + PD, g_next, x_next);
#pragma unroll
    for (int kk = 0; kk < KK; ++kk)
#pragma unroll
      for (int t = 0; t < 3; ++t)
#pragma unroll
        for (int a = 0; a < WM; ++a)
          acc[t][a] = __builtin_amdgcn_mfma_f32_16x16x32_bf16(gf[kk][a], x_frag(kk, t), acc[t][a], 0, 0, 0);
#pragma unroll
    for (int i = 0; i < KK * 3 * WM; ++i) {
      __builtin_amdgcn_sched_group_barrier(0x008, 1, 0);
      __builtin_amdgcn_sched_group_barrier(0x002, 1, 0);
      __builtin_amdgcn_sched_group_barrier(0x004, 1, 0);
    }
#pragma unroll
    for (int kk = 0; kk < KK; ++kk) asm volatile("" : "+v"(xa[kk][0]), "+v"(xa[kk][1]), "+v"(xa[kk][2]));
    asm volatile("" : "+v"(ga[0]), "+v"(ga[1]));
    __builtin_amdgcn_s_setprio(0);
    __builtin_amdgcn_sched_barrier(0);
    __builtin_amdgcn_s_barrier();
    __builtin_amdgcn_sched_barrier(0);
    slot_n = slot_n + 1 == NSLOT ? 0 : slot_n + 1;
    slot_d = slot_d + 1 == NSLOT ? 0 : slot_d + 1;
  }
  for (int i = grp; i < 2; ++i) __builtin_amdgcn_s_barrier();
  const int ci = ci0 + wn * 16 + t16;
#pragma unroll
  for (int t = 0; t < 3; ++t) {
    const int w_tap = d.w_tap[3 * grp + t];
#pragma unroll
    for (int a = 0; a < WM; ++a)
#pragma unroll
      for (int r = 0; r < 4; ++r) {
        const int co = co0 + (wm * WM + a) * 16 + 4 * g4 + r;
        atomicAdd(p.dw + (int64_t)split * p.dw_split_stride + ((int64_t)co * d.w_ntaps + w_tap) * d.cin + ci, acc[t][a][r]);
      }
  }
}

namespace nbdt {

static bool stage_geometry(const nbdt_wgrad_desc* d, int ks, int max_hp, WgradTapsParams* p);

bool wgrad_taps_applicable(const nbdt_wgrad_desc* d) {
  if (d->ntaps != 9 || d->x_base != 0) return false;
  if (d->x_ws != d->cin || d->x_hs != (d->gw + 2) * d->cin || d->x_bs != (d->gh + 2) * d->x_hs) return false;
  for (int t = 0; t < 9; ++t)
    if (d->tap_off[t] != (t / 3) * d->x_hs + (t % 3) * d->x_ws) return false;
  return stage_geometry(d, 32, 128, nullptr);
}

static bool stage_geometry(const nbdt_wgrad_desc* d, int ks, int max_hp, WgradTapsParams* p) {
  const int gw = d->gw, gh = d->gh;
  if (!(gw % ks == 0 || ks % gw == 0)) return false;
  int rs = gw >= ks ? 1 : ks / gw;
  int cs = gw >= ks ? ks : gw;
  if (ks == 64 && gw >= 64 && gw % 32 == 0 && gh % 2 == 0 && (rs + 2) * (cs + 2) > max_hp) {
    rs = 2;
    cs = 32;
  }
  if (gh % rs != 0) return false;
  if ((rs + 2) * (cs + 2) > max_hp) return false;
  const long long M = (long long)d->B * gh * gw;
  if (!p) return true;
  p->stages = (int)(M / ks);
  p->rs = rs; p->cs = cs;
  p->hw2 = cs + 2;
  p->hp = (rs + 2) * (cs + 2);
  p->stages_per_row = gw / cs;
  p->rowgroups = gh / rs;
  p->div_spr = make_fastdiv((unsigned)p->stages_per_row);
  p->div_rg = make_fastdiv((unsigned)p->rowgroups);
  return true;
}

static void split_items(WgradTapsParams& p, int wm, bool pp) {
  const nbdt_wgrad_desc& d = p.d;
  p.n_ci_blocks = d.cin / 32;
  const int tiles = (d.cout / (32 * wm)) * p.n_ci_blocks;
  int cus = d.cu_budget > 0 ? d.cu_budget : 256;
  cus = std::max(8, std::min(cus, 256 - reserved_cus()));
  int splits = (pp ? cus : 2 * cus) / tiles;
  const int max_splits = p.stages / 16 > 0 ? p.stages / 16 : 1;
  if (splits > max_splits) splits = max_splits;
  if (splits < 1) splits = 1;
  p.stages_per_split = (p.stages + splits - 1) / splits;
  splits = (p.stages + p.stages_per_split - 1) / p.stages_per_split;
  p.splits = splits;
  p.items = tiles * splits;
  p.per_xcd = (p.items + 7) / 8;
}
static int cout_tiles_wm(int cout) {
  const int mt = cout / 32;
  return mt % 5 == 0 ? 5 : (mt % 4 == 0 ? 4 : (mt % 2 == 0 ? 2 : 1));
}

template <int WM, int KIND>
static int launch_taps(WgradTapsParams& p, hipStream_t st) {
  constexpr bool PP = KIND != 0;
  split_items(p, WM, PP);
  const size_t shmem = PP ? (size_t)5 * (64 * 64 * WM + 144 * 64) : (size_t)NSTAGE * ((32 * WM / 8) * 512 + x_bytes(4));
  const void* fn = KIND == 3 ? reinterpret_cast<const void*>(&conv_wgrad_ks_kernel<WM>)
                   : KIND == 2 ? reinterpret_cast<const void*>(&conv_wgrad_pp3_kernel<WM>)
                   : KIND == 1 ? reinterpret_cast<const void*>(&conv_wgrad_pp_kernel<WM>)
                               : reinterpret_cast<const void*>(&conv_wgrad_taps_kernel<WM, 4>);
  static DeviceAttr site;
  if (site.need(shmem)) {
    NBDT_ATTR_CHECK(site, hipFuncSetAttribute(fn, hipFuncAttributeMaxDynamicSharedMemorySize, (int)shmem));
    site.done(shmem);
  }
  float* const dw = p.dw;
  const size_t dw_elems = (size_t)p.d.cout * p.d.w_ntaps * p.d.cin;
  p.dw_split_stride = 0;
  bool covers = p.d.w_ntaps == 9;
  {
    unsigned seen = 0;
    for (int t = 0; t < 9; ++t) seen |= 1u << (p.d.w_tap[t] & 31);
    covers = covers && seen == 0x1ffu;
  }
  p.store = (KIND == 3 && covers && ((wgrad_store_epilogue() && p.splits <= 64 && p.d.cu_budget == 0) || deterministic())) ? 1 : 0;
  if (p.store || deterministic()) {
    float* rows = det_rows(st, (size_t)p.splits * dw_elems);
    if (!rows && !deterministic()) {
      p.store = 0;
    } else {
      if (!rows) return nbdt::fail(NBDT_ENOMEM, "weight gradient: %s (%s)", "no workspace for the per-split gradients",
                                   nbdt::det_rows_why());
      if (!p.store) NBDT_HIP_CHECK(hipMemsetAsync(rows, 0, (size_t)p.splits * dw_elems * sizeof(float), st));
      p.dw = rows;
      p.dw_split_stride = (long long)dw_elems;
    }
  }
  void* args[] = {(void*)&p};
  NBDT_HIP_CHECK(hipLaunchKernel(fn, dim3(p.per_xcd * 8), dim3(KIND == 2 ? 768 : (KIND == 0 ? 256 : 512)), args, shmem, st));
  g_last_wgrad = KIND == 3 ? "conv_wgrad_ks_kernel" : KIND == 2 ? "conv_wgrad_pp3_kernel"
                           : (KIND == 1 ? "conv_wgrad_pp_kernel" : "conv_wgrad_taps_kernel");
  if (p.dw != dw) return det_fold(st, p.dw, p.splits, dw_elems, dw);
  return NBDT_OK;
}

static bool pp_fits_shape(const nbdt_wgrad_desc* d) {
  return d->gw % 8 == 0 && stage_geometry(d, 64, 144, nullptr) && (long long)d->B * d->x_bs * 2 < (1ll << 32) &&
         (long long)d->B * d->g_bs * 2 < (1ll << 32);
}
constexpr bool kKsDefault = true;
static bool takes_pp(const nbdt_wgrad_desc* d, bool pp_fits) {
  const long long M = (long long)d->B * d->gh * d->gw;
  constexpr int kMinStages = 64;
  return pp_fits && (d->variant == 2 || d->variant == 4 || d->variant == 5 || (d->variant != 3 && M / 64 >= kMinStages));
}

int wgrad_taps_blocks(const nbdt_wgrad_desc* d) {
  if (!wgrad_taps_applicable(d) || !takes_pp(d, pp_fits_shape(d))) return 0;
  WgradTapsParams p;
  p.d = *d;
  stage_geometry(d, 64, 144, &p);
  split_items(p, cout_tiles_wm(d->cout), true);
  return p.per_xcd * 8 < p.items ? p.per_xcd * 8 : p.items;
}

int wgrad_taps(const nbdt_wgrad_desc* d, const void* x, const void* gy, float* dw, hipStream_t st) {
  WgradTapsParams p;
  p.d = *d;
  p.x = (const bf16_t*)x;
  p.gy = (const bf16_t*)gy;
  p.dw = dw;
  const int mt = d->cout / 32;
  const bool pp_fits = pp_fits_shape(d);
  NBDT_REQUIRE(!((d->variant == 2 || d->variant == 4 || d->variant == 5) && !pp_fits),
               "variant 2 / 4 / 5 (8- / 12-wave / K-split weight-gradient kernel): shape does not fit it");
  const bool pp = takes_pp(d, pp_fits);
  if (pp) {
    stage_geometry(d, 64, 144, &p);
    const bool ksplit = d->variant == 5 || (d->variant == 0 && kKsDefault);
    if (ksplit) {
      if (mt % 5 == 0) return launch_taps<5, 3>(p, st);
      if (mt % 4 == 0) return launch_taps<4, 3>(p, st);
      if (mt % 2 == 0) return launch_taps<2, 3>(p, st);
      return launch_taps<1, 3>(p, st);
    }
    const bool three = d->variant == 4;
    if (three) {
      if (mt % 5 == 0) return launch_taps<5, 2>(p, st);
      if (mt % 4 == 0) return launch_taps<4, 2>(p, st);
      if (mt % 2 == 0) return launch_taps<2, 2>(p, st);
      return launch_taps<1, 2>(p, st);
    }
    if (mt % 5 == 0) return launch_taps<5, 1>(p, st);
    if (mt % 4 == 0) return launch_taps<4, 1>(p, st);
    if (mt % 2 == 0) return launch_taps<2, 1>(p, st);
    return launch_taps<1, 1>(p, st);
  }
  stage_geometry(d, 32, 128, &p);
  if (mt % 5 == 0) return launch_taps<5, 0>(p, st);
  if (mt % 4 == 0) return launch_taps<4, 0>(p, st);
  if (mt % 2 == 0) return launch_taps<2, 0>(p, st);
  return launch_taps<1, 0>(p, st);
}

}
```

### neural-backed-decision-trees_amd/nbdt/_C.py

```python
import ctypes
import os
from ctypes import POINTER, c_char_p, c_float, c_int, c_int32, c_int64, c_void_p

import numpy as np
import torch

_LIBPATH = os.environ.get("NBDT_HIP_LIB") or os.path.join(os.path.dirname(os.path.abspath(__file__)), "_lib",
                                                         "libnbdt_hip.so")
_lib = None

NBDT_F32, NBDT_BF16, NBDT_F16 = 0, 1, 2
NBDT_U8 = 3
NBDT_SD_MAX_UNITS = 64
NBDT_AUGMENT_MAX_PAD = 32
NBDT_RESIZED_CROP_RATIOS = 4096
NBDT_RESIZED_CROP_ATTEMPTS = 10
NBDT_POLICY_NONE, NBDT_POLICY_TA_WIDE = 0, 1
NBDT_POLICY_OPS = 14
NBDT_POLICY_BINS = 31
NBDT_CHAIN_OPS = 15
NBDT_CHAIN_MAX_OPS = 4
NBDT_CHAIN_MAX_BINS = 31
NBDT_CHAIN_MAX_SUBPOLICIES = 1024
NBDT_CHAIN_RAND, NBDT_CHAIN_SUBPOLICY = 0, 1
NBDT_CHAIN_TA_WIDE = 2
NBDT_RESIZED_CROP_POLICY_MAX_SIDE = 512
_ZTYPE = {torch.float32: NBDT_F32, torch.bfloat16: NBDT_BF16, torch.float16: NBDT_F16}


class NBDTHipError(RuntimeError):
    pass


class ConvDesc(ctypes.Structure):
    _fields_ = [
        ("B", c_int32), ("gh", c_int32), ("gw", c_int32),
        ("cin", c_int32), ("cout", c_int32),
        ("ntaps", c_int32),
        ("tap_off", c_int32 * 9), ("w_tap", c_int32 * 9), ("w_ntaps", c_int32),
        ("in_bs", c_int32), ("in_hs", c_int32), ("in_ws", c_int32), ("in_base", c_int32),
        ("out_bs", c_int32), ("out_hs", c_int32), ("out_ws", c_int32), ("out_base", c_int32),
        ("accumulate", c_int32),
        ("wide_tile", c_int32),
        ("ksplit", c_int32),
        ("w_tiled", ctypes.c_uint64),
    ]


class WgradDesc(ctypes.Structure):
    _fields_ = [
        ("B", c_int32), ("gh", c_int32), ("gw", c_int32),
        ("cin", c_int32), ("cout", c_int32),
        ("ntaps", c_int32),
        ("tap_off", c_int32 * 9), ("w_tap", c_int32 * 9), ("w_ntaps", c_int32),
        ("x_bs", c_int32), ("x_hs", c_int32), ("x_ws", c_int32), ("x_base", c_int32),
        ("g_bs", c_int32), ("g_hs", c_int32), ("g_ws", c_int32), ("g_base", c_int32),
        ("variant", c_int32),
        ("cu_budget", c_int32),
    ]


class TreeStats(ctypes.Structure):
    FIELDS = ("totals", "confusion_net", "confusion_hard", "confusion_soft", "node_counts", "node_entropy",
              "first_error_depth")
    _fields_ = [(name, c_void_p) for name in FIELDS]


class ConvSegSlice(ctypes.Structure):
    _fields_ = [("tensor", c_int32), ("ch0", c_int32), ("ntaps", c_int32), ("tap", c_int32 * 9),
                ("w_matrix", c_int32), ("w_off", c_int32 * 9)]


class ConvSegClass(ctypes.Structure):
    _fields_ = [("nslices", c_int32), ("slices", POINTER(ConvSegSlice)),
                ("out_bs", c_int32), ("out_hs", c_int32), ("out_ws", c_int32), ("out_base", c_int32)]


class ConvSegDesc(ctypes.Structure):
    _fields_ = [("B", c_int32), ("gh", c_int32), ("gw", c_int32), ("cout", c_int32),
                ("ntensors", c_int32), ("pix_stride", c_int32 * 4),
                ("nmatrices", c_int32), ("w_row_stride", c_int32 * 4),
                ("nclasses", c_int32), ("cls", ConvSegClass * 4),
                ("tile", c_int32), ("nbuf", c_int32)]


_P = c_void_p
_I32P = POINTER(c_int32)

SIGNATURES = {
    "nbdt_last_error": (c_char_p, []),
    "nbdt_version": (c_int, []),
    "nbdt_device_count": (c_int, []),
    "nbdt_set_deterministic": (c_int, [c_int32]),
    "nbdt_get_deterministic": (c_int, []),
    "nbdt_set_wgrad_store_epilogue": (c_int, [c_int32]),
    "nbdt_get_wgrad_store_epilogue": (c_int, []),
    "nbdt_set_reserved_cus": (c_int, [c_int32]),
    "nbdt_probe_mfma_stream": (c_int, [c_int32, c_int32, _P, _P]),
    "nbdt_probe_lds_mfma": (c_int, [c_int32, c_int32, c_int32, _P, _P]),
    "nbdt_get_reserved_cus": (c_int, []),
    "nbdt_set_stream_nt_min_bytes": (c_int, [c_int64]),
    "nbdt_get_stream_nt_min_bytes": (c_int64, []),
    "nbdt_debug_last_stream_nt": (c_int, []),
    "nbdt_tree_create": (c_int, [c_int, c_int, c_int, c_int, _I32P, _I32P, _I32P, _I32P, _I32P, _I32P,
                                 POINTER(c_void_p)]),
    "nbdt_tree_destroy": (c_int, [c_void_p]),
    "nbdt_tree_max_depth": (c_int, [c_void_p]),
    "nbdt_debug_last_igemm": (c_char_p, []),
    "nbdt_debug_last_igemm_full": (c_char_p, []),
    "nbdt_debug_last_wgrad": (c_char_p, []),
    "nbdt_conv_wgrad_blocks": (c_int, [_P]),
    "nbdt_conv_plan": (c_int, [_P, _P, _P]),
    "nbdt_soft_forward": (c_int, [c_void_p, _P, c_int, c_int64, c_int64, _P, _P]),
    "nbdt_soft_backward": (c_int, [c_void_p, _P, c_int, c_int64, c_int64, _P, _P, _P]),
    "nbdt_soft_tree_loss": (c_int, [c_void_p, _P, c_int, c_int64, c_int64, _P, c_float, c_float, c_float,
                                    _P, _P, _P, _P]),
    "nbdt_head_soft_tree_loss": (c_int, [c_void_p, _P, _P, _P, c_int64, c_int32, _P, c_float, c_float, c_float,
                                         _P, _P, _P, _P, _P, _P, _P]),
    "nbdt_hard_tree_loss": (c_int, [c_void_p, _P, c_int, c_int64, c_int64, _P, c_float, c_float, c_float,
                                    _P, _P, _P, _P]),
    "nbdt_soft_tree_loss_ex": (c_int, [c_void_p, _P, c_int, c_int64, c_int64, _P, _P, c_int64, c_float, c_float, c_float,
                                       c_float, _P, _P, _P, _P]),
    "nbdt_hard_tree_loss_ex": (c_int, [c_void_p, _P, c_int, c_int64, c_int64, _P, c_float, c_float, c_float, c_float,
                                       _P, _P, _P, _P]),
    "nbdt_mix_batch": (c_int, [_P, _P, c_int32, c_int32, c_int32, c_float, c_float, c_int32, c_int32, c_int32, c_int32,
                               c_float, c_float, _P, _P, c_int32, _P]),
    "nbdt_node_logits_backward": (c_int, [c_void_p, _P, c_int64, _P, _P]),
    "nbdt_hard_forward": (c_int, [c_void_p, _P, c_int, c_int64, c_int64, _P, _P, _P, _P, _P, _P, _P]),
    "nbdt_node_outputs": (c_int, [c_void_p, _P, c_int, c_int64, c_int64, _P, _P, _P, _P, _P]),
    "nbdt_tree_stats_accumulate": (c_int, [c_void_p, _P, c_int, c_int64, c_int64, _P, _P, _P, _P]),
    "nbdt_conv_igemm": (c_int, [POINTER(ConvDesc), _P, _P, _P, _P, _P]),
    "nbdt_conv_pw": (c_int, [POINTER(ConvDesc), _P, _P, _P, _P, _P]),
    "nbdt_conv_igemm_multi": (c_int, [_P, c_int32, _P, _P, _P, _P]),
    "nbdt_conv_igemm_stats": (c_int, [POINTER(ConvDesc), _P, _P, _P, _P, _P, _P]),
    "nbdt_conv_seg_create": (c_int, [POINTER(ConvSegDesc), POINTER(c_void_p)]),
    "nbdt_conv_seg_destroy": (c_int, [c_void_p]),
    "nbdt_conv_seg_info": (c_int, [c_void_p, _I32P, _I32P, _I32P, _I32P, POINTER(c_int64)]),
    "nbdt_conv_seg_steps": (c_int, [c_void_p, c_int32, _I32P, c_int32, _I32P]),
    "nbdt_conv_seg_tile_weights": (c_int, [c_void_p, POINTER(c_void_p), _P, _P]),
    "nbdt_conv_seg": (c_int, [c_void_p, POINTER(c_void_p), _P, _P, _P, _P, _P]),
    "nbdt_ref_conv_seg": (c_int, [c_void_p, POINTER(c_void_p), POINTER(c_void_p), _P, _P, _P]),
    "nbdt_bn_apply_s2d": (c_int, [_P, _P, _P, _P, _P, c_int32, c_int32, c_int32, c_int32, c_int32, _P, _P]),
    "nbdt_ref_bn_apply_s2d": (c_int, [_P, _P, _P, _P, _P, c_int32, c_int32, c_int32, c_int32, c_int32, _P, _P]),
    "nbdt_bn_finalize": (c_int, [c_int32, c_int32, c_int32, c_int32, c_float, c_float, _P, _P, _P, _P, _P, _P]),
    "nbdt_conv_igemm_bnbwd": (c_int, [POINTER(ConvDesc), _P, _P, _P, _P, _P, _P, _P, _P, _P, _P]),
    "nbdt_conv_igemm_affine": (c_int, [POINTER(ConvDesc), _P, _P, _P, _P, _P, _P, c_int32, _P]),
    "nbdt_bn_bwd_fold": (c_int, [c_int32, c_int32, c_int32, c_int32, _P, _P, _P, _P, _P]),
    "nbdt_bn_bwd_apply_cus": (c_int, [_P, _P, _P, _P, _P, _P, _P, _P, c_int32, c_int32, c_int32, c_int32, _P, c_int32, _P]),
    "nbdt_bn_bwd_reduce_cus": (c_int, [_P, _P, _P, _P, _P, _P, c_int32, c_int32, c_int32, c_int32, _P, _P, _P, _P, c_int32, _P]),
    "nbdt_bn_bwd_cus": (c_int, [_P, _P, _P, _P, _P, _P, _P, c_int32, c_int32, c_int32, c_int32, _P, _P, _P, _P, _P, _P,
                                c_int32, _P]),
    "nbdt_conv_wgrad": (c_int, [POINTER(WgradDesc), _P, _P, _P, _P]),
    "nbdt_ref_conv": (c_int, [POINTER(ConvDesc), _P, _P, _P, _P, _P]),
    "nbdt_ref_wgrad": (c_int, [POINTER(WgradDesc), _P, _P, _P, _P]),
    "nbdt_ref_bn_stats": (c_int, [_P, c_int32, c_int32, c_int32, c_int32, c_float, c_float, _P, _P, _P, _P, _P, _P]),
    "nbdt_ref_bn_apply": (c_int, [_P, _P, _P, _P, _P, _P, c_int32, c_int32, c_int32, c_int32, c_int32, _P, _P]),
    "nbdt_ref_bn_bwd": (c_int, [_P, _P, _P, _P, _P, _P, _P, _P, c_int32, _P, c_int32, c_int32, c_int32, c_int32,
                                c_int32, _P, _P, _P, _P, _P, _P]),
    "nbdt_ref_bn_relu_pool": (c_int, [_P, _P, _P, _P, _P, c_int32, c_int32, c_int32, c_int32, _P, _P]),
    "nbdt_ref_stem_conv": (c_int, [_P, _P, c_int32, c_int32, c_int32, c_int32, c_int32, c_int32, _P, _P]),
    "nbdt_ref_stem_wgrad": (c_int, [_P, _P, c_int32, c_int32, c_int32, c_int32, c_int32, c_int32, _P, _P]),
    "nbdt_ref_bn_act_apply": (c_int, [_P, _P, _P, _P, _P, c_int32, _P, _P, c_int32, c_int32, c_int32, c_int32, _P, _P]),
    "nbdt_ref_bn_act_pool": (c_int, [_P, _P, _P, _P, _P, c_int32, _P, c_float, c_int32, c_int32, c_int32, c_int32, _P,
                                     _P]),
    "nbdt_ref_bn_act_bwd": (c_int, [_P, _P, _P, _P, _P, _P, _P, _P, c_int32, _P, c_int32, c_int32, c_int32, c_int32, _P,
                                    _P, _P, _P, _P]),
    "nbdt_ref_bn_act_apply_rows": (c_int, [_P, _P, _P, _P, _P, c_int32, _P, _P, _P, c_int32, c_int32, c_int32, c_int32, _P,
                                           _P]),
    "nbdt_ref_bn_act_bwd_rows": (c_int, [_P, _P, _P, _P, _P, _P, _P, _P, _P, c_int32, _P, c_int32, c_int32, c_int32,
                                         c_int32, _P, _P, _P, _P, _P]),
    "nbdt_ref_dwconv_fwd": (c_int, [_P, _P, c_int32, c_int32, c_int32, c_int32, c_int32, c_int32, _P, _P]),
    "nbdt_ref_dwconv_bwd_data": (c_int, [_P, _P, c_int32, c_int32, c_int32, c_int32, c_int32, c_int32, _P, _P]),
    "nbdt_ref_dwconv_bwd_weight": (c_int, [_P, _P, c_int32, c_int32, c_int32, c_int32, c_int32, c_int32, _P, _P]),
    "nbdt_weight_prep": (c_int, [_P, c_int32, c_int32, c_int32, _P, _P, _P]),
    "nbdt_weight_prep_batched": (c_int, [_P, _P, c_int32, c_int64, _P, _P]),
    "nbdt_weight_tile_batched": (c_int, [_P, _P, c_int32, c_int64, _P, _P]),
    "nbdt_bn_stats": (c_int, [_P, c_int32, c_int32, c_int32, c_int32, c_float, c_float, _P, _P, _P, _P, _P, _P]),
    "nbdt_bn_apply": (c_int, [_P, _P, _P, _P, _P, _P, c_int32, c_int32, c_int32, c_int32, c_int32, _P, _P]),
    "nbdt_bn_bwd_reduce": (c_int, [_P, _P, _P, _P, _P, _P, _P, c_int32, c_int32, c_int32, c_int32, c_int32,
                                   _P, _P, _P, _P, _P]),
    "nbdt_bn_bwd_apply": (c_int, [_P, _P, _P, _P, _P, _P, _P, _P, _P, c_int32, c_int32, c_int32, c_int32,
                                  c_int32, _P, _P, _P]),
    "nbdt_bn_relu_pool": (c_int, [_P, _P, _P, _P, _P, c_int32, c_int32, c_int32, c_int32, _P, _P]),
    "nbdt_pool_bn_bwd_reduce": (c_int, [_P, _P, _P, _P, _P, _P, c_int32, c_int32, c_int32, c_int32, _P, _P,
                                        _P, _P, _P]),
    "nbdt_pool_bn_bwd_apply": (c_int, [_P, _P, _P, _P, _P, _P, _P, c_int32, c_int32, c_int32, c_int32, _P,
                                       _P]),
    "nbdt_stem_conv": (c_int, [_P, _P, c_int32, c_int32, c_int32, c_int32, c_int32, c_int32, _P, _P]),
    "nbdt_stem_wgrad": (c_int, [_P, _P, c_int32, c_int32, c_int32, c_int32, c_int32, c_int32, _P, _P]),
    "nbdt_bn_act_apply": (c_int, [_P, _P, _P, _P, _P, c_int32, _P, _P, c_int32, c_int32, c_int32, c_int32, _P, _P]),
    "nbdt_bn_act_pool": (c_int, [_P, _P, _P, _P, _P, c_int32, _P, c_float, c_int32, c_int32, c_int32, c_int32,
                                 _P, _P]),
    "nbdt_bn_act_bwd": (c_int, [_P, _P, _P, _P, _P, _P, _P, _P, c_int32, _P, c_int32, c_int32, c_int32, c_int32,
                                _P, _P, _P, _P, _P, _P]),
    "nbdt_dwconv_fwd": (c_int, [_P, _P, c_int32, c_int32, c_int32, c_int32, c_int32, c_int32, _P, _P, _P]),
    "nbdt_dwconv_bwd_data": (c_int, [_P, _P, c_int32, c_int32, c_int32, c_int32, c_int32, c_int32, _P, _P]),
    "nbdt_dwconv_bwd_data_bn": (c_int, [_P, _P, c_int32, c_int32, c_int32, c_int32, c_int32, _P, _P, _P, _P, _P, _P, _P, _P]),
    "nbdt_bn_act_bwd_apply": (c_int, [_P, _P, _P, _P, _P, _P, c_int32, _P, c_int32, c_int32, c_int32, c_int32,
                                      _P, _P, _P, _P, _P, _P]),
    "nbdt_bn_act_se_sums": (c_int, [_P, _P, _P, _P, _P, _P, c_int32, c_int32, c_int32, c_int32, c_int32, _P, _P]),
    "nbdt_bn_act_se_bwd_apply": (c_int, [_P, _P, _P, _P, _P, _P, _P, _P, _P, c_int32, c_int32, c_int32, c_int32, c_int32,
                                         _P, _P, _P, _P, _P]),
    "nbdt_dwconv_bwd_weight": (c_int, [_P, _P, c_int32, c_int32, c_int32, c_int32, c_int32, c_int32, _P, _P]),
    "nbdt_se_gate_fwd": (c_int, [_P, _P, _P, _P, _P, c_int32, c_int32, c_int32, c_int32, _P, _P, _P]),
    "nbdt_se_gate_bwd": (c_int, [_P, _P, _P, _P, _P, _P, c_int32, c_int32, c_int32, c_int32, _P, _P, _P, _P, _P,
                                 _P, _P, _P]),
    "nbdt_se_param_grad": (c_int, [_P, _P, _P, _P, c_int32, c_int32, c_int32, c_int32, _P, _P, _P, _P, _P]),
    "nbdt_dropout_fwd": (c_int, [_P, c_int64, c_float, ctypes.c_uint32, _P, _P, _P]),
    "nbdt_dropout_bwd": (c_int, [_P, c_int64, c_float, _P, _P, _P]),
    "nbdt_bn_act_apply_rows": (c_int, [_P, _P, _P, _P, _P, c_int32, _P, _P, _P, c_int32, c_int32, c_int32, c_int32, _P,
                                       _P]),
    "nbdt_bn_act_bwd_rows": (c_int, [_P, _P, _P, _P, _P, _P, _P, _P, _P, c_int32, _P, c_int32, c_int32, c_int32, c_int32,
                                     _P, _P, _P, _P, _P, _P]),
    "nbdt_stochastic_depth_draw": (c_int, [ctypes.c_uint64, ctypes.c_uint64, ctypes.c_uint64, POINTER(c_float),
                                           POINTER(c_float), c_int32, c_int32, _P, _P]),
    "nbdt_augment_batch": (c_int, [_P, c_int32, _P, _P, c_int32, c_int64, c_int32, c_int32, c_int32, c_int32,
                                   POINTER(c_float), POINTER(c_float), POINTER(c_float), ctypes.c_uint64, ctypes.c_uint64,
                                   _P, _P, _P, _P, _P]),
    "nbdt_resized_crop_batch": (c_int, [_P, c_int32, _P, _P, c_int32, c_int64] + [c_int32] * 9 +
                                [POINTER(c_float), POINTER(c_float), POINTER(ctypes.c_double), POINTER(ctypes.c_double), _P,
                                 ctypes.c_uint64, ctypes.c_uint64, _P, _P, _P, _P, _P]),
    "nbdt_resized_crop_band_rows": (c_int, [c_int32] * 8),
    "nbdt_augment_batch_sharded": (c_int, [_P, c_int32, _P, _P, c_int64, c_int32, c_int64, c_int32, c_int32, c_int32, c_int32,
                                           POINTER(c_float), POINTER(c_float), POINTER(c_float), ctypes.c_uint64,
                                           ctypes.c_uint64, _P, _P, _P, _P, _P]),
    "nbdt_resized_crop_batch_sharded": (c_int, [_P, c_int32, _P, _P, c_int64, c_int32, c_int64] + [c_int32] * 9 +
                                        [POINTER(c_float), POINTER(c_float), POINTER(ctypes.c_double),
                                         POINTER(ctypes.c_double), _P, ctypes.c_uint64, ctypes.c_uint64, _P, _P, _P, _P, _P]),
    "nbdt_policy_batch": (c_int, [_P, c_int32, _P, _P, c_int32, c_int64, c_int32, c_int32, c_int32, c_int32,
                                  POINTER(c_float), POINTER(c_float), c_int32, _P, ctypes.c_double,
                                  POINTER(ctypes.c_double), POINTER(ctypes.c_double), _P, ctypes.c_uint64, ctypes.c_uint64,
                                  _P, _P, _P, _P, _P, _P, _P]),
    "nbdt_policy_batch_sharded": (c_int, [_P, c_int32, _P, _P, c_int64, c_int32, c_int64, c_int32, c_int32, c_int32,
                                          c_int32, POINTER(c_float), POINTER(c_float), c_int32, _P, ctypes.c_double,
                                          POINTER(ctypes.c_double), POINTER(ctypes.c_double), _P, ctypes.c_uint64,
                                          ctypes.c_uint64, _P, _P, _P, _P, _P, _P, _P]),
    "nbdt_policy_chain_batch": (c_int, [_P, c_int32, _P, _P, c_int32, c_int64, c_int32, c_int32, c_int32, c_int32,
                                        POINTER(c_float), POINTER(c_float), c_int32, c_int32, _P, c_int32, c_int32, _P,
                                        c_int32, ctypes.c_double, POINTER(ctypes.c_double), POINTER(ctypes.c_double), _P,
                                        ctypes.c_uint64, ctypes.c_uint64, _P, _P, _P, _P, _P, _P, _P, _P, _P]),
    "nbdt_policy_chain_batch_sharded": (c_int, [_P, c_int32, _P, _P, c_int64, c_int32, c_int64, c_int32, c_int32, c_int32,
                                                c_int32, POINTER(c_float), POINTER(c_float), c_int32, c_int32, _P, c_int32,
                                                c_int32, _P, c_int32, ctypes.c_double, POINTER(ctypes.c_double),
                                                POINTER(ctypes.c_double), _P, ctypes.c_uint64, ctypes.c_uint64, _P, _P, _P,
                                                _P, _P, _P, _P, _P, _P]),
    "nbdt_resized_crop_policy_batch": (c_int, [_P, c_int32, _P, _P, c_int32, c_int64, c_int32, c_int32, c_int32, c_int32,
                                               POINTER(c_float), POINTER(c_float), POINTER(ctypes.c_double),
                                               POINTER(ctypes.c_double), _P, c_int32, c_int32, _P, c_int32, c_int32, _P,
                                               c_int32, ctypes.c_double, POINTER(ctypes.c_double), POINTER(ctypes.c_double),
                                               _P, ctypes.c_uint64, ctypes.c_uint64] + [_P] * 11),
    "nbdt_resized_crop_policy_batch_sharded": (c_int, [_P, c_int32, _P, _P, c_int64, c_int32, c_int64, c_int32, c_int32,
                                                       c_int32, c_int32, POINTER(c_float), POINTER(c_float),
                                                       POINTER(ctypes.c_double), POINTER(ctypes.c_double), _P, c_int32,
                                                       c_int32, _P, c_int32, c_int32, _P, c_int32, ctypes.c_double,
                                                       POINTER(ctypes.c_double), POINTER(ctypes.c_double), _P,
                                                       ctypes.c_uint64, ctypes.c_uint64] + [_P] * 11),
    "nbdt_stem_patches": (c_int, [_P, c_int32, c_int32, c_int32, c_int32, c_int32, c_int32, c_int32, _P, _P]),
    "nbdt_maxpool3x3s2_fwd": (c_int, [_P, c_int32, c_int32, c_int32, c_int32, c_int32, _P, _P, _P]),
    "nbdt_maxpool3x3s2_bwd": (c_int, [_P, _P, c_int32, c_int32, c_int32, c_int32, c_int32, _P, _P]),
    "nbdt_linear_fwd": (c_int, [_P, _P, _P, c_int32, c_int32, c_int32, _P, _P]),
    "nbdt_linear_bwd": (c_int, [_P, _P, _P, c_int32, c_int32, c_int32, _P, _P, _P, _P]),
    "nbdt_sgd_step": (c_int, [_P, _P, _P, c_int64, c_float, c_float, c_float, c_float, _P, c_int32, _P]),
    "nbdt_lars_create": (c_int, [c_int64, POINTER(c_int64), POINTER(c_int64), POINTER(c_float), _I32P, c_int32,
                                 POINTER(c_void_p)]),
# ... 267 lines not shown
```

### neural-backed-decision-trees_amd/nbdt/ops.py

```python
import contextlib
import ctypes

import numpy as np
import torch

from nbdt import _C
from nbdt._C import ConvDesc, WgradDesc, check, lib, ptr

BN_SLOTS = 32
BN_EPS = 1e-5
BN_MOMENTUM = 0.1


def set_deterministic(on):
    check(lib().nbdt_set_deterministic(1 if on else 0))


def is_deterministic():
    return bool(lib().nbdt_get_deterministic())


def set_wgrad_store_epilogue(on):
    check(lib().nbdt_set_wgrad_store_epilogue(1 if on else 0))

# ... 194 lines not shown
            d["launches"] += 1
            d["flops"] += flops
            d["ms"] += s.elapsed_time(e)
        for d in out.values():
            d["avg_us"] = 1e3 * d["ms"] / max(d["launches"], 1)
            d["tflops"] = d["flops"] / (d["ms"] * 1e-3) / 1e12 if d["ms"] > 0 else 0.0
        return out


_timer = None


def set_timer(t):
    global _timer
    _timer = t



def conv_igemm(desc, inp, w_bf16, out, residual=None, bn_scratch=None):
    if _ref(inp):
        check(lib().nbdt_ref_conv(ctypes.byref(desc), ptr(inp), ptr(w_bf16), ptr(out), ptr(residual),
                                  stream_ptr(inp.device)))
        if bn_scratch is not None:
            B, H, W, C = _dims(out)
            check(lib().nbdt_ref_bn_stats(ptr(out), B, H, W, C, BN_EPS, BN_MOMENTUM, None, None, None, None,
                                          ptr(bn_scratch), stream_ptr(inp.device)))
        return
    ev = None
    if _timer is not None and _timer.wants("conv_igemm"):
        flops = desc_flops(desc)
        ev = _timer.bracket("conv_igemm", flops, inp.device)
        ev[0].record()
    if bn_scratch is None:
        check(lib().nbdt_conv_igemm(ctypes.byref(desc), ptr(inp), ptr(w_bf16), ptr(out), ptr(residual),
                                    stream_ptr(inp.device)))
    else:
        check(lib().nbdt_conv_igemm_stats(ctypes.byref(desc), ptr(inp), ptr(w_bf16), ptr(out), ptr(residual),
                                          ptr(bn_scratch), stream_ptr(inp.device)))
    if ev is not None:
        ev[1].record()
        _timer.count(last_igemm_kernel_full())


def conv_pw(desc, inp, w_bf16, out, bn_scratch=None):
    if _ref(inp):
        conv_igemm(desc, inp, w_bf16, out, None, bn_scratch)
        return
    ev = None
    if _timer is not None and _timer.wants("conv_igemm"):
        flops = desc_flops(desc)
        ev = _timer.bracket("conv_igemm", flops, inp.device)
        ev[0].record()
    check(lib().nbdt_conv_pw(ctypes.byref(desc), ptr(inp), ptr(w_bf16), ptr(out), ptr(bn_scratch),
                             stream_ptr(inp.device)))
    if ev is not None:
        ev[1].record()
        _timer.count(last_igemm_kernel_full())


def desc_flops(desc):
    cin, cout = getattr(desc, "flop_channels", (desc.cin, desc.cout))
    return 2.0 * desc.B * desc.gh * desc.gw * desc.ntaps * cin * cout


def conv_igemm_multi(descs, inp, w_bf16, out):
    if _ref(inp):
        for d in descs:
            check(lib().nbdt_ref_conv(ctypes.byref(d), ptr(inp), ptr(w_bf16), ptr(out), None, stream_ptr(inp.device)))
        return
    arr = (ConvDesc * len(descs))(*descs)
    ev = None
    if _timer is not None and _timer.wants("conv_igemm"):
        flops = sum(desc_flops(d) for d in descs)
        ev = _timer.bracket("conv_igemm", flops, inp.device)
        ev[0].record()
    check(lib().nbdt_conv_igemm_multi(arr, len(descs), ptr(inp), ptr(w_bf16), ptr(out), stream_ptr(inp.device)))
    if ev is not None:
        ev[1].record()
        _timer.count(last_igemm_kernel_full())


def conv_igemm_bnbwd(desc, inp, w_bf16, out, bn_x, mean, rstd, gamma, beta, partials):
    _no_ref(inp, "conv_igemm_bnbwd (fused BatchNorm-backward sums): use the split or the unfused schedule")
    ev = None
    if _timer is not None and _timer.wants("conv_igemm"):
        flops = desc_flops(desc)
        ev = _timer.bracket("conv_igemm", flops, inp.device)
        ev[0].record()
    check(lib().nbdt_conv_igemm_bnbwd(ctypes.byref(desc), ptr(inp), ptr(w_bf16), ptr(out), ptr(bn_x), ptr(mean),
                                      ptr(rstd), ptr(gamma), ptr(beta), ptr(partials), stream_ptr(inp.device)))
    if ev is not None:
        ev[1].record()
        _timer.count(last_igemm_kernel_full())


def conv_igemm_affine(desc, inp, w_bf16, out, scale, shift, act=1, residual=None):
    _no_ref(inp, "conv_igemm_affine (folded eval-mode BatchNorm): engine.fuse_eval is off in reference mode")
    check(lib().nbdt_conv_igemm_affine(ctypes.byref(desc), ptr(inp), ptr(w_bf16), ptr(out), ptr(residual),
                                       ptr(scale), ptr(shift), act, stream_ptr(inp.device)))


def bn_bwd_fused(gy, x, mean, rstd, gamma, beta, partials, dsum, dgamma, dbeta, gx, gx_add=None, cus=0):
    _no_ref(x, "bn_bwd_fused: use the split or the unfused schedule")
    B, H, W, C = _dims(x)
    st = stream_ptr(x.device)
    check(lib().nbdt_bn_bwd_fold(B, H, W, C, ptr(partials), ptr(dsum), ptr(dgamma), ptr(dbeta), st))
    if cus > 0:
        check(lib().nbdt_bn_bwd_apply_cus(ptr(gy), ptr(x), ptr(mean), ptr(rstd), ptr(gamma), ptr(beta), ptr(dsum),
                                          ptr(gx_add), B, H, W, C, ptr(gx), int(cus), st))
        return
    check(lib().nbdt_bn_bwd_apply(ptr(gy), None, ptr(x), ptr(mean), ptr(rstd), ptr(gamma), ptr(beta),
                                  ptr(dsum), ptr(gx_add), 1, B, H, W, C, ptr(gx), None, st))


def bn_bwd_cus(gy, x, mean, rstd, gamma, beta, scratch, dsum, dgamma, dbeta, gx, cus, gx_add=None):
    B, H, W, C = _dims(x)
    st = stream_ptr(x.device)
    if _ref(x):
        check(lib().nbdt_ref_bn_bwd(ptr(gy), None, None, ptr(x), ptr(mean), ptr(rstd), ptr(gamma), ptr(beta), 1,
                                    ptr(gx_add), B, H, W, C, 1, ptr(dsum), ptr(dgamma), ptr(dbeta), ptr(gx), None, st))
        return
    if isinstance(scratch, (tuple, list)):
        slots, other = scratch
        check(lib().nbdt_bn_bwd_cus(ptr(gy), ptr(x), ptr(mean), ptr(rstd), ptr(gamma), ptr(beta), ptr(gx_add), B, H, W,
                                    C, ptr(slots), ptr(other), ptr(dsum), ptr(dgamma), ptr(dbeta), ptr(gx), int(cus),
                                    st))
        return
    check(lib().nbdt_bn_bwd_reduce_cus(ptr(gy), ptr(x), ptr(mean), ptr(rstd), ptr(gamma), ptr(beta), B, H, W, C,
                                       ptr(scratch), ptr(dsum), ptr(dgamma), ptr(dbeta), int(cus), st))
    check(lib().nbdt_bn_bwd_apply_cus(ptr(gy), ptr(x), ptr(mean), ptr(rstd), ptr(gamma), ptr(beta), ptr(dsum),
                                      ptr(gx_add), B, H, W, C, ptr(gx), int(cus), st))


def conv_wgrad(desc, x, gy, dw, cu_budget=0):
    desc.cu_budget = int(cu_budget)
    if _ref(x):
        check(lib().nbdt_ref_wgrad(ctypes.byref(desc), ptr(x), ptr(gy), ptr(dw), stream_ptr(x.device)))
        return
    ev = None
    if _timer is not None and _timer.wants("conv_wgrad"):
        flops = desc_flops(desc)
        ev = _timer.bracket("conv_wgrad", flops, x.device)
        ev[0].record()
    check(lib().nbdt_conv_wgrad(ctypes.byref(desc), ptr(x), ptr(gy), ptr(dw), stream_ptr(x.device)))
    if ev is not None:
        ev[1].record()


def conv_wgrad_blocks(desc, cu_budget=0):
    desc.cu_budget = int(cu_budget)
    return int(lib().nbdt_conv_wgrad_blocks(ctypes.byref(desc)))


MI355X_CUS, MI355X_XCDS = 256, 8


def cu_topology_is_mi355x(device):
    props = torch.cuda.get_device_properties(device)
    return props.multi_processor_count == MI355X_CUS and "gfx950" in getattr(props, "gcnArchName", "gfx950")


def plan_cu_share(desc, elements, tensors, gbps_per_cu, target_us, min_cus, max_cus):
    held = (reserved_cus() + MI355X_XCDS - 1) // MI355X_XCDS
    per_xcd = MI355X_CUS // MI355X_XCDS - held
    cus = per_xcd * MI355X_XCDS
    n = int(round(elements * 2 * tensors / (gbps_per_cu * 1e9 * target_us * 1e-6)))
    n = max(max(8, int(min_cus)), min(int(max_cus), n))
    n = min(n, cus - MI355X_XCDS)
    while True:
        blocks = conv_wgrad_blocks(desc, cus - n)
        if not 0 < blocks <= cus - n:
            return cus - n, n
        free = MI355X_XCDS * (per_xcd - (blocks + MI355X_XCDS - 1) // MI355X_XCDS)
        if free >= MI355X_XCDS or n + MI355X_XCDS > cus - MI355X_XCDS:
            return cus - n, max(free, MI355X_XCDS)
        n += MI355X_XCDS


def weight_prep(w_fp32, cout, taps, cin, w_bf16=None, wd_bf16=None):
    check(lib().nbdt_weight_prep(ptr(w_fp32), cout, taps, cin, ptr(w_bf16), ptr(wd_bf16),
                                 stream_ptr(w_fp32.device)))


def weight_tile_batched(src_bf16, table, n, total, dst_bf16):
    check(lib().nbdt_weight_tile_batched(ptr(src_bf16), ptr(table), n, total, ptr(dst_bf16),
                                         stream_ptr(src_bf16.device)))


def weight_tiles(w_bf16):
    rows, taps, k = w_bf16.shape
    assert taps == 9 and rows % 32 == 0 and k % 32 == 0
    r32 = rows // 32
    nt = 5 if r32 % 5 == 0 else 4 if r32 % 4 == 0 else 2 if r32 % 2 == 0 else 1
    total = (rows // (32 * nt)) * (k // 32) * 9
    table = torch.tensor([[0, 0, rows, k, 0]], dtype=torch.int64, device=w_bf16.device)
    dst = torch.empty(rows * 9 * k, dtype=torch.bfloat16, device=w_bf16.device)
    weight_tile_batched(w_bf16.contiguous(), table, 1, total, dst)
    return dst


def last_igemm_kernel():
    return lib().nbdt_debug_last_igemm().decode()


def last_igemm_kernel_full():
    return lib().nbdt_debug_last_igemm_full().decode()


def last_wgrad_kernel():
    return lib().nbdt_debug_last_wgrad().decode()


def weight_prep_batched(flat, table, n_layers, total, wd_flat):
    check(lib().nbdt_weight_prep_batched(ptr(flat), ptr(table), n_layers, total, ptr(wd_flat),
                                         stream_ptr(flat.device)))


def _dims(t):
    B, Hp, Wp, C = t.shape
    return B, Hp - 2, Wp - 2, C


def bn_stats(x, scratch, save_mean, save_rstd, running_mean=None, running_var=None,
             eps=BN_EPS, momentum=BN_MOMENTUM, slots_filled=False):
    B, H, W, C = _dims(x)
    if _ref(x):
        check(lib().nbdt_ref_bn_stats(ptr(x), B, H, W, C, eps, momentum, ptr(running_mean), ptr(running_var),
                                      ptr(save_mean), ptr(save_rstd), None, stream_ptr(x.device)))
        return
    check(lib().nbdt_bn_stats(None if slots_filled else ptr(x), B, H, W, C, eps, momentum, ptr(running_mean), ptr(running_var),
                              ptr(scratch), ptr(save_mean), ptr(save_rstd), stream_ptr(x.device)))


def bn_finalize(x, scratch, save_mean, save_rstd, running_mean=None, running_var=None,
                eps=BN_EPS, momentum=BN_MOMENTUM):
    B, H, W, C = _dims(x)
    check(lib().nbdt_bn_finalize(B, H, W, C, eps, momentum, ptr(running_mean), ptr(running_var), ptr(scratch),
                                 ptr(save_mean), ptr(save_rstd), stream_ptr(x.device)))


def bn_apply(x, mean, rstd, gamma, beta, y, relu=True, residual=None):
    B, H, W, C = _dims(x)
    if _ref(x):
        check(lib().nbdt_ref_bn_apply(ptr(x), ptr(mean), ptr(rstd), ptr(gamma), ptr(beta), ptr(residual),
                                      1 if relu else 0, B, H, W, C, ptr(y), stream_ptr(x.device)))
        return
    check(lib().nbdt_bn_apply(ptr(x), ptr(mean), ptr(rstd), ptr(gamma), ptr(beta), ptr(residual),
                              1 if relu else 0, B, H, W, C, ptr(y), stream_ptr(x.device)))


def bn_bwd(gy, y, x, mean, rstd, gamma, scratch, dsum, dgamma, dbeta, gx, relu=True, gx_add=None,
           g_resid=None, beta=None):
    B, H, W, C = _dims(x)
    st = stream_ptr(x.device)
    r = 1 if relu else 0
    if _ref(x):
        check(lib().nbdt_ref_bn_bwd(ptr(gy), None, ptr(y), ptr(x), ptr(mean), ptr(rstd), ptr(gamma), ptr(beta), r,
                                    ptr(gx_add), B, H, W, C, 1, ptr(dsum), ptr(dgamma), ptr(dbeta), ptr(gx), ptr(g_resid),
                                    st))
        return
    check(lib().nbdt_bn_bwd_reduce(ptr(gy), ptr(y), ptr(x), ptr(mean), ptr(rstd), ptr(gamma), ptr(beta), r,
                                   B, H, W, C, ptr(scratch), ptr(dsum), ptr(dgamma), ptr(dbeta), st))
    check(lib().nbdt_bn_bwd_apply(ptr(gy), ptr(y), ptr(x), ptr(mean), ptr(rstd), ptr(gamma), ptr(beta),
                                  ptr(dsum), ptr(gx_add), r, B, H, W, C, ptr(gx), ptr(g_resid), st))


def bn_relu_pool(x, mean, rstd, gamma, beta, pooled):
    B, H, W, C = _dims(x)
    if _ref(x):
        check(lib().nbdt_ref_bn_relu_pool(ptr(x), ptr(mean), ptr(rstd), ptr(gamma), ptr(beta), B, H, W, C, ptr(pooled),
                                          stream_ptr(x.device)))
        return
    check(lib().nbdt_bn_relu_pool(ptr(x), ptr(mean), ptr(rstd), ptr(gamma), ptr(beta), B, H, W, C,
                                  ptr(pooled), stream_ptr(x.device)))


def pool_bn_bwd(gpooled, x, mean, rstd, gamma, beta, scratch, dsum, dgamma, dbeta, gx):
    B, H, W, C = _dims(x)
    st = stream_ptr(x.device)
    if _ref(x):
        check(lib().nbdt_ref_bn_bwd(None, ptr(gpooled), None, ptr(x), ptr(mean), ptr(rstd), ptr(gamma), ptr(beta), 1,
                                    None, B, H, W, C, 1, ptr(dsum), ptr(dgamma), ptr(dbeta), ptr(gx), None, st))
        return
    check(lib().nbdt_pool_bn_bwd_reduce(ptr(gpooled), ptr(x), ptr(mean), ptr(rstd), ptr(gamma), ptr(beta),
                                        B, H, W, C, ptr(scratch), ptr(dsum), ptr(dgamma), ptr(dbeta), st))
    check(lib().nbdt_pool_bn_bwd_apply(ptr(gpooled), ptr(x), ptr(mean), ptr(rstd), ptr(gamma), ptr(beta),
                                       ptr(dsum), B, H, W, C, ptr(gx), st))


def pool_bn_bwd_apply(gpooled, x, mean, rstd, gamma, beta, dsum, gx):
    B, H, W, C = _dims(x)
    st = stream_ptr(x.device)
    if _ref(x):
        check(lib().nbdt_ref_bn_bwd(None, ptr(gpooled), None, ptr(x), ptr(mean), ptr(rstd), ptr(gamma), ptr(beta), 1,
                                    None, B, H, W, C, 0, ptr(dsum), None, None, ptr(gx), None, st))
        return
    check(lib().nbdt_pool_bn_bwd_apply(ptr(gpooled), ptr(x), ptr(mean), ptr(rstd), ptr(gamma), ptr(beta), ptr(dsum),
                                       B, H, W, C, ptr(gx), st))


def stem_conv(img, w, out, cout_real, stride=1):
    B, _, H, W = img.shape
    if _ref(out):
        check(lib().nbdt_ref_stem_conv(ptr(img), ptr(w), B, H, W, cout_real, out.shape[3], stride, ptr(out),
                                       stream_ptr(img.device)))
        return
# ... 790 lines not shown
```

Baseline: 31980 images/sec.

## Persist wgrad DMA blocks under CU budget, batch BN loads, model single-tile CU count

The DMA weight-gradient kernel becomes grid-strided over work items, so the grid can be capped at the CU budget while each block processes several tiles. A shared plan function is exposed to Python for inspection. BN stats and apply kernels for narrow channel counts (C<=64) now issue four loads before consuming them, to raise memory-level parallelism. A cost model picks the CU count for single-tile pipelined taps wgrad, trading HBM streaming time against atomic reduction traffic. A scratch timing script is added. Risks include extra register pressure from the batched loads and idle CUs when the cost model undershoots.

```diff
diff --git a/include/nbdt_hip.h b/include/nbdt_hip.h
--- a/include/nbdt_hip.h
+++ b/include/nbdt_hip.h
@@ -168,6 +168,7 @@
 int nbdt_conv_wgrad(const nbdt_wgrad_desc* d, const void* x, const void* gy, float* dw,
                     void* stream);
 int nbdt_conv_wgrad_blocks(const nbdt_wgrad_desc* d);
+int nbdt_conv_wgrad_dma_plan(const nbdt_wgrad_desc* d, int32_t* splits, int32_t* chunks_per_split, int32_t* blocks);
 
 int nbdt_weight_prep(const float* w, int32_t cout, int32_t taps, int32_t cin, void* w_bf16,
                      void* wd_bf16, void* stream);
diff --git a/neural-backed-decision-trees_amd/csrc/bn.hip b/neural-backed-decision-trees_amd/csrc/bn.hip
--- a/neural-backed-decision-trees_amd/csrc/bn.hip
+++ b/neural-backed-decision-trees_amd/csrc/bn.hip
@@ -16,6 +16,8 @@
   l.threads = l.c8 * l.py;
   return l;
 }
+constexpr int kStreamInFlight = 4;
+static bool small_c(int C) { return C <= 64; }
 static int grid_for(const PadGeom& g, const Layout& l, int pixels_per_thread) {
   long long want = ((long long)g.npix + (long long)l.py * pixels_per_thread - 1) / ((long long)l.py * pixels_per_thread);
   if (want < 1) want = 1;
@@ -44,14 +46,13 @@
 
 __global__ __launch_bounds__(kMaxThreads) void bn_stats_kernel(const bf16_t* __restrict__ x, PadGeom g, int c8,
                                                                int PY, float* __restrict__ scratch,
-                                                               unsigned slot_mask) {
+                                                               unsigned slot_mask, int batched) {
   extern __shared__ float lds[];
   const int cx = threadIdx.x % c8, py = threadIdx.x / c8;
   float acc[2][8];
 #pragma unroll
   for (int i = 0; i < 8; ++i) acc[0][i] = acc[1][i] = 0.f;
-  for (int p = blockIdx.x * PY + py; p < g.npix; p += gridDim.x * PY) {
-    const u32x4_t v = *(const u32x4_t*)(x + pad_offset(g, p) + cx * 8);
+  auto one = [&](const u32x4_t v) {
     float f[8];
     unpack8(v, f);
 #pragma unroll
@@ -59,7 +60,17 @@
       acc[0][i] += f[i];
       acc[1][i] += f[i] * f[i];
     }
-  }
+  };
+  const int step = gridDim.x * PY;
+  int p = blockIdx.x * PY + py;
+  for (; batched && p + (kStreamInFlight - 1) * step < g.npix; p += kStreamInFlight * step) {
+    u32x4_t v[kStreamInFlight];
+#pragma unroll
+    for (int u = 0; u < kStreamInFlight; ++u) v[u] = *(const u32x4_t*)(x + pad_offset(g, p + u * step) + cx * 8);
+#pragma unroll
+    for (int u = 0; u < kStreamInFlight; ++u) one(v[u]);
+  }
+  for (; p < g.npix; p += step) one(*(const u32x4_t*)(x + pad_offset(g, p) + cx * 8));
   block_fold_to_slots<2>(acc, cx, py, c8, PY, g.C, scratch, lds, slot_mask);
 }
 
@@ -124,7 +135,7 @@
                                                                const float* __restrict__ gamma,
                                                                const float* __restrict__ beta,
                                                                const bf16_t* __restrict__ res, PadGeom g, int c8,
-                                                               int PY, bf16_t* __restrict__ y) {
+                                                               int PY, bf16_t* __restrict__ y, int batched) {
   const int cx = threadIdx.x % c8, py = threadIdx.x / c8;
   float sc[8], sh[8];
 #pragma unroll
@@ -133,12 +144,10 @@
     sc[i] = gamma[c] * rstd[c];
     sh[i] = beta[c] - mean[c] * sc[i];
   }
-  for (int p = blockIdx.x * PY + py; p < g.npix; p += gridDim.x * PY) {
-    const int o = pad_offset(g, p) + cx * 8;
-    float f[8];
-    unpack8(ld16_stream<NT>(x + o), f);
-    float r[8];
-    if (HAS_RES) unpack8(ld16_stream<NT>(res + o), r);
+  auto one = [&](int o, const u32x4_t vx, const u32x4_t vr) {
+    float f[8], r[8];
+    unpack8(vx, f);
+    if (HAS_RES) unpack8(vr, r);
 #pragma unroll
     for (int i = 0; i < 8; ++i) {
       float v = f[i] * sc[i] + sh[i];
@@ -147,6 +156,28 @@
       f[i] = v;
     }
     *(u32x4_t*)(y + o) = pack8(f);
+  };
+  const int step = gridDim.x * PY;
+  int p = blockIdx.x * PY + py;
+  for (; batched && p + (kStreamInFlight - 1) * step < g.npix; p += kStreamInFlight * step) {
+    int o[kStreamInFlight];
+    u32x4_t vx[kStreamInFlight], vr[kStreamInFlight];
+#pragma unroll
+    for (int u = 0; u < kStreamInFlight; ++u) {
+      o[u] = pad_offset(g, p + u * step) + cx * 8;
+      vx[u] = ld16_stream<NT>(x + o[u]);
+      vr[u] = vx[u];
+      if (HAS_RES) vr[u] = ld16_stream<NT>(res + o[u]);
+    }
+#pragma unroll
+    for (int u = 0; u < kStreamInFlight; ++u) one(o[u], vx[u], vr[u]);
+  }
+  for (; p < g.npix; p += step) {
+    const int o = pad_offset(g, p) + cx * 8;
+    const u32x4_t vx = ld16_stream<NT>(x + o);
+    u32x4_t vr = vx;
+    if (HAS_RES) vr = ld16_stream<NT>(res + o);
+    one(o, vx, vr);
   }
 }
 
@@ -529,7 +560,7 @@
     rc = slot_target(st, scratch, grid, 2 * (size_t)C, &t);
     if (rc) return rc;
     hipLaunchKernelGGL(bn_stats_kernel, dim3(grid), dim3(l.threads), shmem, st, (const bf16_t*)x, g,
-                       l.c8, l.py, t.ptr, t.mask);
+                       l.c8, l.py, t.ptr, t.mask, small_c(C) ? 1 : 0);
     NBDT_LAUNCH_CHECK();
     rc = slot_finish(st, t, grid, 2 * (size_t)C, scratch);
     if (rc) return rc;
@@ -669,9 +700,9 @@
 #define NBDT_APPLY(R, S)                                                                                         \
   do {                                                                                                           \
     if (nt) hipLaunchKernelGGL((bn_apply_kernel<R, S, true>), grid, blk, 0, st, (const bf16_t*)x, save_mean, save_rstd, gamma, \
-                               beta, (const bf16_t*)residual, g, l.c8, l.py, (bf16_t*)y);                          \
+                               beta, (const bf16_t*)residual, g, l.c8, l.py, (bf16_t*)y, small_c(C) ? 1 : 0);                          \
     else hipLaunchKernelGGL((bn_apply_kernel<R, S, false>), grid, blk, 0, st, (const bf16_t*)x, save_mean, save_rstd, gamma, \
-                            beta, (const bf16_t*)residual, g, l.c8, l.py, (bf16_t*)y);                             \
+                            beta, (const bf16_t*)residual, g, l.c8, l.py, (bf16_t*)y, small_c(C) ? 1 : 0);                             \
   } while (0)
   if (relu) { if (residual) NBDT_APPLY(true, true); else NBDT_APPLY(true, false); }
   else { if (residual) NBDT_APPLY(false, true); else NBDT_APPLY(false, false); }
diff --git a/neural-backed-decision-trees_amd/csrc/common.h b/neural-backed-decision-trees_amd/csrc/common.h
--- a/neural-backed-decision-trees_amd/csrc/common.h
+++ b/neural-backed-decision-trees_amd/csrc/common.h
@@ -146,6 +146,7 @@
 }
 
 int wgrad_dma(const nbdt_wgrad_desc* d, const void* x, const void* gy, float* dw, hipStream_t st);
+void wgrad_dma_plan(const nbdt_wgrad_desc* d, int* splits, int* chunks_per_split, int* blocks);
 
 bool wgrad_taps_applicable(const nbdt_wgrad_desc* d);
 int wgrad_taps(const nbdt_wgrad_desc* d, const void* x, const void* gy, float* dw, hipStream_t st);
diff --git a/neural-backed-decision-trees_amd/csrc/rules.hip b/neural-backed-decision-trees_amd/csrc/rules.hip
--- a/neural-backed-decision-trees_amd/csrc/rules.hip
+++ b/neural-backed-decision-trees_amd/csrc/rules.hip
@@ -1300,7 +1300,7 @@
 
 
 extern "C" const char* nbdt_last_error(void) { return nbdt::g_err; }
-extern "C" int nbdt_version(void) { return 124; }
+extern "C" int nbdt_version(void) { return 125; }
 extern "C" int nbdt_device_count(void) {
   int n = 0;
   if (hipGetDeviceCount(&n) != hipSuccess) return 0;
diff --git a/neural-backed-decision-trees_amd/csrc/wgrad.hip b/neural-backed-decision-trees_amd/csrc/wgrad.hip
--- a/neural-backed-decision-trees_amd/csrc/wgrad.hip
+++ b/neural-backed-decision-trees_amd/csrc/wgrad.hip
@@ -33,5 +33,19 @@
   return nbdt::wgrad_taps_blocks(d);
 }
 
+extern "C" int nbdt_conv_wgrad_dma_plan(const nbdt_wgrad_desc* d, int32_t* splits, int32_t* chunks_per_split,
+                                        int32_t* blocks) {
+  NBDT_REQUIRE(d && splits && chunks_per_split && blocks, "null argument");
+  NBDT_REQUIRE(d->cin > 0 && d->cin % 32 == 0 && d->cout > 0 && d->cout % 32 == 0, "channels must be multiples of 32");
+  NBDT_REQUIRE(d->ntaps >= 1 && d->ntaps <= 9, "bad tap table");
+  NBDT_REQUIRE(d->B > 0 && d->gh > 0 && d->gw > 0, "empty pixel grid");
+  NBDT_REQUIRE(d->cu_budget == 0 || (d->cu_budget >= 32 && d->cu_budget <= 256), "cu_budget must be 0 or 32..256");
+  NBDT_REQUIRE((int64_t)d->B * d->gh * d->gw < (1ll << 31), "pixel grid too large");
+  int s = 0, c = 0, b = 0;
+  nbdt::wgrad_dma_plan(d, &s, &c, &b);
+  *splits = s; *chunks_per_split = c; *blocks = b;
+  return NBDT_OK;
+}
+
 namespace nbdt { thread_local const char* g_last_wgrad = ""; }
 extern "C" const char* nbdt_debug_last_wgrad(void) { return nbdt::g_last_wgrad; }
diff --git a/neural-backed-decision-trees_amd/csrc/wgrad_dma.hip b/neural-backed-decision-trees_amd/csrc/wgrad_dma.hip
--- a/neural-backed-decision-trees_amd/csrc/wgrad_dma.hip
+++ b/neural-backed-decision-trees_amd/csrc/wgrad_dma.hip
@@ -1,5 +1,6 @@
 #include "common.h"
 #include <stdlib.h>
+#include <algorithm>
 
 using namespace nbdt;
 
@@ -20,6 +21,7 @@
   int chunks_per_split;
   int n_ci_blocks;
   int splits, items, per_xcd;
+  int grid;
   FastDiv div_gw, div_gh;
 };
 
@@ -67,22 +69,6 @@
   const int lane = tid & 63;
   const int wave = __builtin_amdgcn_readfirstlane(tid >> 6);
   const int wm = wave >> 1, wn = wave & 1;
-
-  const int item = (blockIdx.x & 7) * p.per_xcd + (blockIdx.x >> 3);
-  if (item >= p.items) return;
-  const int tap = item % d.ntaps;
-  const int rest = item / d.ntaps;
-  const int split = rest % p.splits;
-  const int tile = rest / p.splits;
-  const int co_blk = tile / p.n_ci_blocks;
-  const int ci_blk = tile - co_blk * p.n_ci_blocks;
-  const int co0 = co_blk * CG;
-  const int ci0 = ci_blk * CX;
-  const int c_begin = split * p.chunks_per_split;
-  int c_end = c_begin + p.chunks_per_split;
-  c_end = c_end < p.chunks ? c_end : p.chunks;
-  if (c_begin >= c_end) return;
-  const int n_chunks = c_end - c_begin;
 
 #define NBDT_PIN(x) __builtin_amdgcn_readfirstlane(x)
   const int M = NBDT_PIN(p.M);
@@ -100,44 +86,7 @@
 
   const int hi_half = lane >> 5;
   const int my_px = (lane & 31) ^ (hi_half << 3);
-  const int g_base_off = d.g_base + co0 + hi_half * 8;
-  const int x_base_off = d.x_base + d.tap_off[tap] + ci0 + hi_half * 8;
-  const int g_zero = co0 + hi_half * 8;
-  const int x_zero = ci0 + hi_half * 8;
   const unsigned lds_base = (unsigned)(size_t)(__attribute__((address_space(3))) unsigned char*)smem;
-
-  auto issue = [&](int slot, int chunk) {
-    const int m = chunk * KS + my_px;
-    const bool valid = m < M;
-    const unsigned mm = valid ? (unsigned)m : 0u;
-    const unsigned t1 = fdiv(mm, dgw);
-    const int j = (int)(mm - t1 * dgw.d);
-    const unsigned b = fdiv(t1, dgh);
-    const int i = (int)(t1 - b * dgh.d);
-    const int og = valid ? ((int)b * g_bs + i * g_hs + j * g_ws + g_base_off) : g_zero;
-    const int ox = valid ? ((int)b * x_bs + i * x_hs + j * x_ws + x_base_off) : x_zero;
-    const bf16_t* gsrc = gy_base + og;
-    const bf16_t* xsrc = x_base + ox;
-    const unsigned dst0 = lds_base + slot * STAGE;
-#pragma unroll
-    for (int k = 0; k < IPG; ++k) {
-      const int id = wave + 4 * k;
-      if (id < G_INSTR)
-        glds16(gsrc + id * 16, __builtin_amdgcn_readfirstlane(dst0 + id * 1024));
-    }
-#pragma unroll
-    for (int k = 0; k < IPX; ++k) {
-      const int id = ((wave + 2) & 3) + 4 * k;
-      if (id < X_INSTR)
-        glds16(xsrc + id * 16, __builtin_amdgcn_readfirstlane(dst0 + G_BYTES + id * 1024));
-    }
-  };
-
-  f32x4 acc[WM][WN];
-#pragma unroll
-  for (int a = 0; a < WM; ++a)
-#pragma unroll
-    for (int b = 0; b < WN; ++b) acc[a][b] = f32x4{0.f, 0.f, 0.f, 0.f};
 
   const int g4 = lane >> 4, t16 = lane & 15;
   const int rr = 4 * g4 + (t16 >> 2);
@@ -153,71 +102,172 @@
     return bf16x8{lo[0], lo[1], lo[2], lo[3], hi[0], hi[1], hi[2], hi[3]};
   };
 
-  auto compute = [&](int slot) {
-    const unsigned char* Gs = smem + slot * STAGE + g_lane_off;
-    const unsigned char* Xs = smem + slot * STAGE + G_BYTES + x_lane_off;
-    bf16x8 gf[WM];
-#pragma unroll
-    for (int a = 0; a < WM; ++a) gf[a] = frag(Gs, a);
-#pragma unroll
-    for (int b = 0; b < WN; ++b) {
-      const bf16x8 xf = frag(Xs, b);
-#pragma unroll
-      for (int a = 0; a < WM; ++a)
-        acc[a][b] = __builtin_amdgcn_mfma_f32_16x16x32_bf16(gf[a], xf, acc[a][b], 0, 0, 0);
+  const int n_slots = p.per_xcd * 8;
+  for (int vb = blockIdx.x; vb < n_slots; vb += gridDim.x) {
+    const int item = (vb & 7) * p.per_xcd + (vb >> 3);
+    if (item >= p.items) continue;
+    const int tap = item % d.ntaps;
+    const int rest = item / d.ntaps;
+    const int split = rest % p.splits;
+    const int tile = rest / p.splits;
+    const int co_blk = tile / p.n_ci_blocks;
+    const int ci_blk = tile - co_blk * p.n_ci_blocks;
+    const int co0 = co_blk * CG;
+    const int ci0 = ci_blk * CX;
+    const int c_begin = split * p.chunks_per_split;
+    int c_end = c_begin + p.chunks_per_split;
+    c_end = c_end < p.chunks ? c_end : p.chunks;
+    if (c_begin >= c_end) continue;
+    const int n_chunks = c_end - c_begin;
+
+    const int g_base_off = d.g_base + co0 + hi_half * 8;
+    const int x_base_off = d.x_base + d.tap_off[tap] + ci0 + hi_half * 8;
+    const int g_zero = co0 + hi_half * 8;
+    const int x_zero = ci0 + hi_half * 8;
+
+    auto issue = [&](int slot, int chunk) {
+      const int m = chunk * KS + my_px;
+      const bool valid = m < M;
+      const unsigned mm = valid ? (unsigned)m : 0u;
+      const unsigned t1 = fdiv(mm, dgw);
+      const int j = (int)(mm - t1 * dgw.d);
+      const unsigned b = fdiv(t1, dgh);
+      const int i = (int)(t1 - b * dgh.d);
+      const int og = valid ? ((int)b * g_bs + i * g_hs + j * g_ws + g_base_off) : g_zero;
+      const int ox = valid ? ((int)b * x_bs + i * x_hs + j * x_ws + x_base_off) : x_zero;
+      const bf16_t* gsrc = gy_base + og;
+      const bf16_t* xsrc = x_base + ox;
+      const unsigned dst0 = lds_base + slot * STAGE;
+#pragma unroll
+      for (int k = 0; k < IPG; ++k) {
+        const int id = wave + 4 * k;
+        if (id < G_INSTR)
+          glds16(gsrc + id * 16, __builtin_amdgcn_readfirstlane(dst0 + id * 1024));
+      }
+#pragma unroll
+      for (int k = 0; k < IPX; ++k) {
+        const int id = ((wave + 2) & 3) + 4 * k;
+        if (id < X_INSTR)
+          glds16(xsrc + id * 16, __builtin_amdgcn_readfirstlane(dst0 + G_BYTES + id * 1024));
+      }
+    };
+
+    f32x4 acc[WM][WN];
+#pragma unroll
+    for (int a = 0; a < WM; ++a)
+#pragma unroll
+      for (int b = 0; b < WN; ++b) acc[a][b] = f32x4{0.f, 0.f, 0.f, 0.f};
+
+    auto compute = [&](int slot) {
+      const unsigned char* Gs = smem + slot * STAGE + g_lane_off;
+      const unsigned char* Xs = smem + slot * STAGE + G_BYTES + x_lane_off;
+      bf16x8 gf[WM];
+#pragma unroll
+      for (int a = 0; a < WM; ++a) gf[a] = frag(Gs, a);
+#pragma unroll
+      for (int b = 0; b < WN; ++b) {
+        const bf16x8 xf = frag(Xs, b);
+#pragma unroll
+        for (int a = 0; a < WM; ++a)
+          acc[a][b] = __builtin_amdgcn_mfma_f32_16x16x32_bf16(gf[a], xf, acc[a][b], 0, 0, 0);
+      }
+    };
+
+    issue(0, c_begin);
+    if (n_chunks > 1) issue(1, c_begin + 1);
+    int slot = 0;
+    for (int t = 0; t < n_chunks; ++t) {
+      if (t + 1 < n_chunks) {
+        asm volatile("s_waitcnt vmcnt(%0) lgkmcnt(0)" ::"n"(MINPW) : "memory");
+      } else {
+        asm volatile("s_waitcnt vmcnt(0) lgkmcnt(0)" ::: "memory");
+      }
+      __builtin_amdgcn_s_barrier();
+      asm volatile("" ::: "memory");
+      if (t + 2 < n_chunks) {
+        int s2 = slot + 2;
+        s2 = s2 >= NSTAGE ? s2 - NSTAGE : s2;
+        issue(s2, c_begin + t + 2);
+      }
+      compute(slot);
+      slot = slot + 1 == NSTAGE ? 0 : slot + 1;
     }
-  };
-
-  issue(0, c_begin);
-  if (n_chunks > 1) issue(1, c_begin + 1);
-  int slot = 0;
-  for (int t = 0; t < n_chunks; ++t) {
-    if (t + 1 < n_chunks) {
-      asm volatile("s_waitcnt vmcnt(%0) lgkmcnt(0)" ::"n"(MINPW) : "memory");
-    } else {
-      asm volatile("s_waitcnt vmcnt(0) lgkmcnt(0)" ::: "memory");
+
+    const int w_tap = d.w_tap[tap];
+#pragma unroll
+    for (int a = 0; a < WM; ++a)
+#pragma unroll
+      for (int b = 0; b < WN; ++b) {
+        const int ci = ci0 + (wn * WN + b) * 16 + t16;
+#pragma unroll
+        for (int r = 0; r < 4; ++r) {
+          const int co = co0 + (wm * WM + a) * 16 + 4 * g4 + r;
+          atomicAdd(p.dw + (int64_t)split * p.dw_split_stride + ((int64_t)co * d.w_ntaps + w_tap) * d.cin + ci, acc[a][b][r]);
+        }
+      }
+    if (vb + (int)gridDim.x < n_slots) {
+      asm volatile("s_waitcnt lgkmcnt(0)" ::: "memory");
+      __builtin_amdgcn_s_barrier();
+      asm volatile("" ::: "memory");
     }
-    __builtin_amdgcn_s_barrier();
-    asm volatile("" ::: "memory");
-    if (t + 2 < n_chunks) {
-      int s2 = slot + 2;
-      s2 = s2 >= NSTAGE ? s2 - NSTAGE : s2;
-      issue(s2, c_begin + t + 2);
+  }
+}
+
+namespace nbdt {
+
+static int tile32(int n32) { return n32 % 5 == 0 ? 5 : n32 % 4 == 0 ? 4 : n32 % 3 == 0 ? 3 : n32 % 2 == 0 ? 2 : 1; }
+
+static void plan_dma(WgradDmaParams& p, int wm, int wn) {
+  constexpr double kHbmBps = 5.0e12, kDmaLatency = 1.1e-6, kAtomicBpsPerCu = 256.0 / 50e-9;
+  const nbdt_wgrad_desc& d = p.d;
+  p.n_ci_blocks = d.cin / (32 * wn);
+  const int tiles = d.ntaps * (d.cout / (32 * wm)) * p.n_ci_blocks;
+  int cus = d.cu_budget > 0 ? d.cu_budget : 256;
+  cus = std::max(8, std::min(cus, 256 - reserved_cus()));
+  const double tile_bytes = 32.0 * wm * 32.0 * wn * 4.0;
+  const double stage_bytes = (32.0 * wm + 32.0 * wn) * KS * 2.0;
+  const double traffic = (double)p.M * tiles * (32.0 * wm + 32.0 * wn) * 2.0;
+  const int max_splits = std::max(1, p.chunks / 16);
+  const int first = (d.cu_budget > 0 || d.ntaps == 1) ? 1 : 2, last = d.cu_budget > 0 ? 1 : 2;
+  double best = 0.;
+  p.splits = 0;
+  for (int per_cu = first; per_cu <= last; ++per_cu) {
+    const int slots = per_cu * cus;
+    int splits = std::max(1, std::min(slots / tiles, max_splits));
+    const int cps = (p.chunks + splits - 1) / splits;
+    splits = (p.chunks + cps - 1) / cps;
+    const int blocks = tiles * splits;
+    const int resident = std::min(blocks, slots);
+    const int rounds = (blocks + slots - 1) / slots;
+    const int on_cu = std::min(per_cu, (resident + cus - 1) / cus);
+    const double cost = traffic / std::min(kHbmBps, resident * 2.0 * stage_bytes / kDmaLatency) +
+                        rounds * on_cu * tile_bytes / kAtomicBpsPerCu;
+    if (p.splits == 0 || cost < best) {
+      best = cost;
+      p.splits = splits;
+      p.chunks_per_split = cps;
     }
-    compute(slot);
-    slot = slot + 1 == NSTAGE ? 0 : slot + 1;
-  }
-
-  const int w_tap = d.w_tap[tap];
-#pragma unroll
-  for (int a = 0; a < WM; ++a)
-#pragma unroll
-    for (int b = 0; b < WN; ++b) {
-      const int ci = ci0 + (wn * WN + b) * 16 + t16;
-#pragma unroll
-      for (int r = 0; r < 4; ++r) {
-        const int co = co0 + (wm * WM + a) * 16 + 4 * g4 + r;
-        atomicAdd(p.dw + (int64_t)split * p.dw_split_stride + ((int64_t)co * d.w_ntaps + w_tap) * d.cin + ci, acc[a][b][r]);
-      }
-    }
-}
-
-namespace nbdt {
+  }
+  p.items = tiles * p.splits;
+  p.per_xcd = (p.items + 7) / 8;
+  p.grid = p.per_xcd * 8;
+  if (d.cu_budget > 0 && p.grid > cus) p.grid = cus & ~7;
+}
+
+void wgrad_dma_plan(const nbdt_wgrad_desc* d, int* splits, int* chunks_per_split, int* blocks) {
+  WgradDmaParams p;
+  p.d = *d;
+  p.M = d->B * d->gh * d->gw;
+  p.chunks = (p.M + KS - 1) / KS;
+  plan_dma(p, tile32(d->cout / 32), tile32(d->cin / 32));
+  *splits = p.splits;
+  *chunks_per_split = p.chunks_per_split;
+  *blocks = std::min(p.grid, p.items);
+}
 
 template <int WM, int WN>
 static int launch_dma(WgradDmaParams& p, hipStream_t st) {
-  const nbdt_wgrad_desc& d = p.d;
-  p.n_ci_blocks = d.cin / (32 * WN);
-  const int tiles = d.ntaps * (d.cout / (32 * WM)) * p.n_ci_blocks;
-  int splits = 512 / tiles;
-  const int max_splits = p.chunks / 16 > 0 ? p.chunks / 16 : 1;
-  if (splits > max_splits) splits = max_splits;
-  if (splits < 1) splits = 1;
-  p.chunks_per_split = (p.chunks + splits - 1) / splits;
-  splits = (p.chunks + p.chunks_per_split - 1) / p.chunks_per_split;
-  p.splits = splits;
-  p.items = tiles * splits;
-  p.per_xcd = (p.items + 7) / 8;
+  plan_dma(p, WM, WN);
   const size_t shmem = (size_t)NSTAGE * (32 * WM / 8 + 32 * WN / 8) * 512;
   static DeviceAttr site;
   if (site.need(shmem)) {
@@ -235,7 +285,7 @@
     p.dw = rows;
     p.dw_split_stride = (long long)dw_elems;
   }
-  hipLaunchKernelGGL((conv_wgrad_dma_kernel<WM, WN>), dim3(p.per_xcd * 8), dim3(256), shmem, st, p);
+  hipLaunchKernelGGL((conv_wgrad_dma_kernel<WM, WN>), dim3(p.grid), dim3(256), shmem, st, p);
   NBDT_LAUNCH_CHECK();
   if (p.dw != dw) return det_fold(st, p.dw, p.splits, dw_elems, dw);
   return NBDT_OK;
diff --git a/neural-backed-decision-trees_amd/csrc/wgrad_taps.hip b/neural-backed-decision-trees_amd/csrc/wgrad_taps.hip
--- a/neural-backed-decision-trees_amd/csrc/wgrad_taps.hip
+++ b/neural-backed-decision-trees_amd/csrc/wgrad_taps.hip
@@ -1085,12 +1085,26 @@
   return true;
 }
 
+static int single_tile_cus(int stages, int wm, int max_cus) {
+  constexpr double kHbmBps = 3.7e12, kAtomicBps = 1.3e12, kCuFlops = 0.6 * 2.5e15 / 256;
+  const double tile_bytes = 32.0 * wm * 32.0 * 9.0 * 4.0, stage_bytes = 64.0 * (32.0 * wm + 32.0) * 2.0;
+  const double stage_s = 2.0 * 64.0 * 32.0 * wm * 32.0 * 9.0 / kCuFlops;
+  int best_cus = max_cus;
+  double best = 0.;
+  for (int c = std::min(64, max_cus); c <= max_cus; c += 8) {
+    const int sps = (stages + c - 1) / c, splits = (stages + sps - 1) / sps;
+    const double cost = std::max(stages * stage_bytes / kHbmBps, sps * stage_s) + splits * tile_bytes / kAtomicBps;
+    if (c == std::min(64, max_cus) || cost < best) { best = cost; best_cus = c; }
+  }
+  return best_cus;
+}
 static void split_items(WgradTapsParams& p, int wm, bool pp) {
   const nbdt_wgrad_desc& d = p.d;
   p.n_ci_blocks = d.cin / 32;
   const int tiles = (d.cout / (32 * wm)) * p.n_ci_blocks;
   int cus = d.cu_budget > 0 ? d.cu_budget : 256;
   cus = std::max(8, std::min(cus, 256 - reserved_cus()));
+  if (pp && tiles == 1 && d.cu_budget == 0) cus = single_tile_cus(p.stages, wm, cus);
   int splits = (pp ? cus : 2 * cus) / tiles;
   const int max_splits = p.stages / 16 > 0 ? p.stages / 16 : 1;
   if (splits > max_splits) splits = max_splits;
diff --git a/neural-backed-decision-trees_amd/nbdt/_C.py b/neural-backed-decision-trees_amd/nbdt/_C.py
--- a/neural-backed-decision-trees_amd/nbdt/_C.py
+++ b/neural-backed-decision-trees_amd/nbdt/_C.py
@@ -110,6 +110,7 @@
     "nbdt_debug_last_igemm_full": (c_char_p, []),
     "nbdt_debug_last_wgrad": (c_char_p, []),
     "nbdt_conv_wgrad_blocks": (c_int, [_P]),
+    "nbdt_conv_wgrad_dma_plan": (c_int, [_P, _P, _P, _P]),
     "nbdt_conv_plan": (c_int, [_P, _P, _P]),
     "nbdt_soft_forward": (c_int, [c_void_p, _P, c_int, c_int64, c_int64, _P, _P]),
     "nbdt_soft_backward": (c_int, [c_void_p, _P, c_int, c_int64, c_int64, _P, _P, _P]),
diff --git a/neural-backed-decision-trees_amd/nbdt/ops.py b/neural-backed-decision-trees_amd/nbdt/ops.py
--- a/neural-backed-decision-trees_amd/nbdt/ops.py
+++ b/neural-backed-decision-trees_amd/nbdt/ops.py
@@ -370,6 +370,13 @@
     return int(lib().nbdt_conv_wgrad_blocks(ctypes.byref(desc)))
 
 
+def conv_wgrad_dma_plan(desc, cu_budget=0):
+    desc.cu_budget = int(cu_budget)
+    s, c, b = ctypes.c_int32(0), ctypes.c_int32(0), ctypes.c_int32(0)
+    check(lib().nbdt_conv_wgrad_dma_plan(ctypes.byref(desc), ctypes.byref(s), ctypes.byref(c), ctypes.byref(b)))
+    return s.value, c.value, b.value
+
+
 MI355X_CUS, MI355X_XCDS = 256, 8
 
 
diff --git a/scratch/time_narrow_launches.py b/scratch/time_narrow_launches.py
--- /dev/null
+++ b/scratch/time_narrow_launches.py
@@ -0,0 +1,85 @@
+#!/usr/bin/env python3
+import os
+import sys
+
+HERE = os.path.dirname(os.path.dirname(os.path.abspath(__file__)))
+ROOT = os.environ.get("NBDT_TREE", HERE)
+sys.path.insert(0, ROOT)
+os.chdir(ROOT)
+import nbdt_path
+
+nbdt_path.add()
+import torch
+from nbdt import ops
+
+DEV = "cuda:0"
+tag = sys.argv[1] if len(sys.argv) > 1 else "x"
+
+
+def med(fn, n=20, warm=3):
+    for _ in range(warm):
+        fn()
+    torch.cuda.synchronize()
+    ts = []
+    for _ in range(n):
+        e0, e1 = torch.cuda.Event(enable_timing=True), torch.cuda.Event(enable_timing=True)
+        e0.record()
+        fn()
+        e1.record()
+        e1.synchronize()
+        ts.append(e0.elapsed_time(e1) * 1e3)
+    ts.sort()
+    return ts[len(ts) // 2], ts[0], ts[-1]
+
+
+def rnd(*shape):
+    return (torch.randn(*shape, device=DEV) * 0.5).to(torch.bfloat16)
+
+
+def report(name, t):
+    print(f"{tag} {name:58s} median {t[0]:8.1f} us  min {t[1]:8.1f}  max {t[2]:8.1f}", flush=True)
+
+
+def wgrad_case(name, desc, xshape, gshape, budgets=(0,)):
+    x, gy = rnd(*xshape), rnd(*gshape)
+    dw = torch.zeros(desc.cout * desc.w_ntaps * desc.cin, device=DEV)
+    for b in budgets:
+        try:
+            t = med(lambda: ops.conv_wgrad(desc, x, gy, dw, b))
+            report(f"{name} budget {b} [{ops.last_wgrad_kernel()}]", t)
+        except Exception as e:
+            print(f"{tag} {name} budget {b}: {e}", flush=True)
+
+
+B = 512
+for (hi, cin, cout) in ((32, 160, 320), (16, 320, 640)):
+    ho = hi // 2
+    d = ops.conv_wgrad_desc_s2d(B, hi, hi, cin, cout, 1)
+    wgrad_case(f"shortcut s2d {cin}->{cout} {ho}x{ho}", d, (B, ho + 2, ho + 2, 4 * cin), (B, ho + 2, ho + 2, cout),
+               budgets=(0, 160, 200))
+d = ops.conv_wgrad_desc(B, 32, 32, 32, 160, 1, 1)
+wgrad_case("first-unit shortcut 32->160 32x32", d, (B, 34, 34, 32), (B, 34, 34, 160), budgets=(0, 160, 200))
+d = ops.conv_wgrad_desc(B, 32, 32, 32, 160, 3, 1)
+wgrad_case("first-unit conv1 3x3 32->160 32x32", d, (B, 34, 34, 32), (B, 34, 34, 160), budgets=(0, 96, 128, 160, 192, 224))
+
+for C, bb in ((32, 512), (64, 128)):
+    x, gy, y, gx = rnd(bb, 34, 34, C), rnd(bb, 34, 34, C), rnd(bb, 34, 34, C), rnd(bb, 34, 34, C)
+    scratch = torch.zeros(32 * 2 * C, device=DEV)
+    mean, rstd = torch.zeros(C, device=DEV), torch.ones(C, device=DEV)
+    gamma, beta = torch.ones(C, device=DEV), torch.zeros(C, device=DEV)
+    dsum, dg, db = torch.zeros(2 * C, device=DEV), torch.zeros(C, device=DEV), torch.zeros(C, device=DEV)
+    report(f"bn_stats(+finalize) C={C} B={bb}", med(lambda: ops.bn_stats(x, scratch, mean, rstd)))
+    mean.zero_(); rstd.fill_(1.0)
+    report(f"bn_apply relu C={C} B={bb}", med(lambda: ops.bn_apply(x, mean, rstd, gamma, beta, y, relu=True)))
+    report(f"bn_bwd (reduce+finalize+apply) C={C} B={bb}",
+           med(lambda: ops.bn_bwd(gy, None, x, mean, rstd, gamma, scratch, dsum, dg, db, gx, relu=True, beta=beta)))
+
+sys.path.insert(0, os.path.join(HERE, "tests"))
+import _resnet_conv_cases as RC
+
+for case in RC.RESNET_CASES:
+    _, H, W, cin, cout, k, stride = case
+    if RC.kernel_names(case)[2] != "conv_wgrad_dma_kernel":
+        continue
+    d = ops.conv_wgrad_desc(128, H, W, cin, cout, k, stride)
+    wgrad_case("resnet " + RC.case_id(case), d, (128, H + 2, W + 2, cin), (128, H // stride + 2, W // stride + 2, cout))
```

After: 31960 images/sec. No clear change (-0.1%).
